# learningmatter-mit/surface-sampling

Measured on AMD Instinct MI355X. Metric: MC energy-evaluations/sec (SrTiO3(001) ~250-atom slabs, 3-model PaiNN ensemble E+F incl. neighbor list), higher is better.
Workload: dtype f32 via fp16x2-split MFMA (3 products), fp32 accumulate; neighbor decisions f64; 1 GPU; SrTiO3(001) PaiNN x3, 256 batched independent chains per GPU (BASELINE configs[3]), 248-272 atoms/chain; chains_per_gpu=256, atoms_per_gpu=66503, edges_per_gpu=2747786, slots_per_gpu=2836316, models=3, streams_per_gpu=2, parallelism=one GPU, no collective

## Files before the change

### surface-sampling_amd/csrc/api_batch.hip

```cpp
#include <cmath>

#include "vssr_internal.h"

namespace vssr {

static void cell_host_setup(const double *cell, const uint8_t *pbc, double cutoff, double inv[9], int nimg[3],
                            bool &ok) {
    const double *a = cell, *b = cell + 3, *c = cell + 6;
    double bc[3] = {b[1] * c[2] - b[2] * c[1], b[2] * c[0] - b[0] * c[2], b[0] * c[1] - b[1] * c[0]};
    double ca[3] = {c[1] * a[2] - c[2] * a[1], c[2] * a[0] - c[0] * a[2], c[0] * a[1] - c[1] * a[0]};
    double ab[3] = {a[1] * b[2] - a[2] * b[1], a[2] * b[0] - a[0] * b[2], a[0] * b[1] - a[1] * b[0]};
    double vol = a[0] * bc[0] + a[1] * bc[1] + a[2] * bc[2];
    ok = true;
    for (int x = 0; x < 9; ++x) inv[x] = 0.0;
    nimg[0] = nimg[1] = nimg[2] = 0;
    if (!(pbc[0] || pbc[1] || pbc[2])) return;
    if (std::fabs(vol) < 1e-12) { ok = false; return; }
    for (int x = 0; x < 3; ++x) { inv[x] = bc[x] / vol; inv[3 + x] = ca[x] / vol; inv[6 + x] = ab[x] / vol; }
    double hgt[3] = {std::fabs(vol) / std::sqrt(bc[0] * bc[0] + bc[1] * bc[1] + bc[2] * bc[2]),
                     std::fabs(vol) / std::sqrt(ca[0] * ca[0] + ca[1] * ca[1] + ca[2] * ca[2]),
                     std::fabs(vol) / std::sqrt(ab[0] * ab[0] + ab[1] * ab[1] + ab[2] * ab[2])};
    for (int k = 0; k < 3; ++k)
        if (pbc[k]) nimg[k] = (int)std::floor(cutoff / hgt[k]) + 1;
}
// ... 247 lines not shown
        return set_err(h, VSSR_E_BADARG, "bad FIRE parameters");
    VSSR_HIP(h, hipSetDevice(h->device));
    h->relax_regrows = 0;
    h->last_want = want | VSSR_WANT_FORCES;
    if (int rc = relax_fire(h, *params, fixed, want)) return rc;
    return relax_finish(h, pos_out, n_steps, converged);
}

static int relax_finish(vssr_handle *h, double *pos_out, int32_t *n_steps, uint8_t *converged) {
    VSSR_HIP(h, hipStreamSynchronize(h->stream));
    h->prof.collect();
    if (pos_out) VSSR_HIP(h, hipMemcpy(pos_out, h->d_pos.p, sizeof(double) * 3 * h->n_atoms, hipMemcpyDeviceToHost));
    if (n_steps) VSSR_HIP(h, hipMemcpy(n_steps, h->d_relax_steps.p, sizeof(int) * h->n_cfg, hipMemcpyDeviceToHost));
    if (converged) VSSR_HIP(h, hipMemcpy(converged, h->d_relax_conv.p, (size_t)h->n_cfg, hipMemcpyDeviceToHost));
    return VSSR_OK;
}

int vssr_profile_enable(vssr_handle *h, int enable) {
    if (int rc = check_kind(h, KINDS_EVAL, __func__)) return rc;
    VSSR_HIP(h, hipStreamSynchronize(h->stream));
    h->prof.collect();
    h->prof.enabled = enable != 0;
    return VSSR_OK;
}
int vssr_profile_reset(vssr_handle *h) {
    if (int rc = check_kind(h, KINDS_EVAL, __func__)) return rc;
    VSSR_HIP(h, hipStreamSynchronize(h->stream));
    h->prof.reset();
    return VSSR_OK;
}
int vssr_profile_read(vssr_handle *h, int32_t cap, const char **names, int64_t *launches, double *total_ms,
                      int32_t *n_out) {
    if (!h || !n_out) return VSSR_E_BADARG;
    if (int rc = check_kind(h, KINDS_EVAL, __func__)) return rc;
    VSSR_HIP(h, hipStreamSynchronize(h->stream));
    h->prof.collect();
    int n = 0;
    for (int k = 0; k < KC_COUNT && n < cap; ++k) {
        if (names) names[n] = kKernelClassNames[k];
        if (launches) launches[n] = h->prof.launches[k];
        if (total_ms) total_ms[n] = h->prof.total_ms[k];
        ++n;
    }
    *n_out = n;
    return VSSR_OK;
}

int vssr_batch_stats(vssr_handle *h, int64_t *n_atoms, int64_t *n_edges, int64_t *n_slots) {
    if (int rc = check_kind(h, KINDS_EVAL, __func__)) return rc;
    if (!h->ran) return set_err(h, VSSR_E_STATE, "no completed run");
    if (h->graph_partial)
        return set_err(h, VSSR_E_STATE, "the resident graph covers only the chains of the last relaxation iteration: run the batch once (vssr_batch_run) first");
    int rc = sync_and_check(h);
    if (rc) return rc;
    if (n_atoms) *n_atoms = h->n_atoms;
    if (n_edges) *n_edges = h->h_counters[1];
    if (n_slots) *n_slots = h->h_counters[0];
    return VSSR_OK;
}

int vssr_batch_neighbors(vssr_handle *h, int64_t cap, int32_t *ei, int32_t *ej, int32_t *eS, float *er,
                         int64_t *n_edges) {
    if (!h || !n_edges) return VSSR_E_BADARG;
    if (int rc = check_kind(h, KINDS_EVAL, __func__)) return rc;
    if (!h->ran) return set_err(h, VSSR_E_STATE, "no completed run");
    if (h->graph_partial)
        return set_err(h, VSSR_E_STATE, "the resident graph covers only the chains of the last relaxation iteration: run the batch once (vssr_batch_run) first");
    int rc = sync_and_check(h);
    if (rc) return rc;
    const int N = h->n_atoms;
    const int64_t slots = h->h_counters[0];
    *n_edges = h->h_counters[1];
    if (!ei && !ej && !eS && !er) return VSSR_OK;
    std::vector<int> row(N + 1), S(slots), wrap((size_t)3 * N);
    std::vector<float4> edge(slots);
    VSSR_HIP(h, hipMemcpy(row.data(), h->d_row_start.p, sizeof(int) * (N + 1), hipMemcpyDeviceToHost));
    VSSR_HIP(h, hipMemcpy(S.data(), h->d_edge_S.p, sizeof(int) * slots, hipMemcpyDeviceToHost));
    VSSR_HIP(h, hipMemcpy(edge.data(), h->d_edge.p, sizeof(float4) * slots, hipMemcpyDeviceToHost));
    VSSR_HIP(h, hipMemcpy(wrap.data(), h->d_wrap.p, sizeof(int) * 3 * N, hipMemcpyDeviceToHost));
    int64_t n = 0;
    for (int i = 0; i < N; ++i)
        for (int e = row[i]; e < row[i + 1]; ++e) {
            int j;
            memcpy(&j, &edge[e].w, sizeof(int));
            if (j < 0) continue;
            if (n < cap) {
                if (ei) ei[n] = i;
                if (ej) ej[n] = j;
                if (eS)
                    for (int k = 0; k < 3; ++k)
                        eS[3 * n + k] = (((S[e] >> (8 * k)) & 255) - 128) + wrap[3 * i + k] - wrap[3 * j + k];
                if (er) { er[3 * n] = edge[e].x; er[3 * n + 1] = edge[e].y; er[3 * n + 2] = edge[e].z; }
            }
            ++n;
        }
    return VSSR_OK;
}

int vssr_batch_device_results(vssr_handle *h, const float **energy, const float **energy_std) {
    if (int rc = check_kind(h, KINDS_EVAL, __func__)) return rc;
    if (!h->ran || h->kind != Kind::PAINN) return set_err(h, VSSR_E_STATE, "no completed PaiNN run");
    if (energy) *energy = h->d_energy.as<float>();
    if (energy_std) *energy_std = h->d_energy_std.as<float>();
    return VSSR_OK;
}

int vssr_batch_device_results_f64(vssr_handle *h, const double **energy, const double **energy_std) {
    if (int rc = check_kind(h, KINDS_EVAL, __func__)) return rc;
    if (!h->ran || h->kind != Kind::PAINN) return set_err(h, VSSR_E_STATE, "no completed PaiNN run");
    if (energy) *energy = h->d_energy64.as<double>();
    if (energy_std) *energy_std = h->d_energy64.as<double>() + h->n_cfg;
    return VSSR_OK;
}

int vssr_batch_energy_f64(vssr_handle *h, double *energy, double *energy_std, double *energy_models) {
    if (int rc = check_kind(h, KINDS_EVAL, __func__)) return rc;
    if (!h->ran) return set_err(h, VSSR_E_STATE, "vssr_batch_energy_f64 before a run");
    VSSR_HIP(h, hipSetDevice(h->device));
    int rc = sync_and_check(h);
    if (rc) return rc;
    const size_t B = h->n_cfg, M = h->n_models;
    if (is_analytic(h)) {
        if (energy) VSSR_HIP(h, hipMemcpy(energy, h->d_pot_e.p, sizeof(double) * B, hipMemcpyDeviceToHost));
        if (energy_models) VSSR_HIP(h, hipMemcpy(energy_models, h->d_pot_e.p, sizeof(double) * B, hipMemcpyDeviceToHost));
        if (energy_std) for (size_t b = 0; b < B; ++b) energy_std[b] = 0.0;
        return VSSR_OK;
    }
    const double *src = h->d_energy64.as<double>();
    if (energy) VSSR_HIP(h, hipMemcpy(energy, src, sizeof(double) * B, hipMemcpyDeviceToHost));
    if (energy_std) VSSR_HIP(h, hipMemcpy(energy_std, src + B, sizeof(double) * B, hipMemcpyDeviceToHost));
    if (energy_models) VSSR_HIP(h, hipMemcpy(energy_models, src + 2 * B, sizeof(double) * B * M, hipMemcpyDeviceToHost));
    return VSSR_OK;
}

int vssr_batch_results_f64(vssr_handle *h, double *energy, double *energy_atoms, double *forces) {
    if (int rc = check_kind(h, KINDS_EVAL, __func__)) return rc;
    if (!is_analytic(h)) return set_err(h, VSSR_E_STATE, "vssr_batch_results_f64 needs an fp64 potential (Tersoff / EAM / SW / pair handle)");
    if (!h->ran) return set_err(h, VSSR_E_STATE, "vssr_batch_results_f64 before a run");
    VSSR_HIP(h, hipSetDevice(h->device));
    if (forces && !(h->last_want & VSSR_WANT_FORCES))
        return set_err(h, VSSR_E_STATE, "forces requested, but the last run was asked for energies only");
    int rc = sync_and_check(h);
    if (rc) return rc;
    const size_t B = h->n_cfg, N = h->n_atoms;
    if (energy) VSSR_HIP(h, hipMemcpy(energy, h->d_pot_e.p, sizeof(double) * B, hipMemcpyDeviceToHost));
    if (energy_atoms) VSSR_HIP(h, hipMemcpy(energy_atoms, h->d_pot_ea.p, sizeof(double) * N, hipMemcpyDeviceToHost));
    if (forces) VSSR_HIP(h, hipMemcpy(forces, h->d_pot_f.p, sizeof(double) * 3 * N, hipMemcpyDeviceToHost));
    return VSSR_OK;
}

int vssr_device_context(vssr_handle *h, int32_t *device, void **stream, const int32_t **overflow_flag) {
    if (int rc = check_kind(h, KINDS_EVAL, __func__)) return rc;
    if (device) *device = h->device;
    if (stream) *stream = (void *)h->stream;
    if (overflow_flag) *overflow_flag = h->d_counters.p ? h->d_counters.as<int>() + 2 : nullptr;
    return VSSR_OK;
}

int vssr_batch_traj_configure(vssr_handle *h, int32_t record_interval) {
    if (int rc = check_kind(h, KINDS_EVAL, __func__)) return rc;
    if (record_interval < 0) return set_err(h, VSSR_E_BADARG, "record_interval must be >= 0");
    h->traj_interval = record_interval;
    return VSSR_OK;
}

int vssr_batch_traj_read(vssr_handle *h, int32_t cap_records, int32_t *n_records, double *pos, float *forces, double *energy,
                         int32_t *max_records) {
    if (int rc = check_kind(h, KINDS_EVAL, __func__)) return rc;
    if (max_records) *max_records = h->traj_records;
    if (!h->traj_records) {
        if (n_records || pos || forces || energy) return set_err(h, VSSR_E_STATE, "the last relaxation recorded no trajectory");
        return VSSR_OK;
    }
    if (!n_records && !pos && !forces && !energy) return VSSR_OK;
    if (h->traj_B != h->n_cfg || h->traj_N != h->n_atoms) return set_err(h, VSSR_E_STATE, "the recorded trajectory belongs to another batch");
    if (cap_records < h->traj_records) return set_err(h, VSSR_E_BADARG, "trajectory buffers hold %d records, %d are needed", cap_records, h->traj_records);
    VSSR_HIP(h, hipSetDevice(h->device));
    VSSR_HIP(h, hipStreamSynchronize(h->stream));
    const size_t R = h->traj_records, N3 = (size_t)3 * h->traj_N, B = h->traj_B;
    if (n_records) VSSR_HIP(h, hipMemcpy(n_records, h->d_traj_n.p, sizeof(int) * B, hipMemcpyDeviceToHost));
    if (pos) VSSR_HIP(h, hipMemcpy(pos, h->d_traj_pos.p, sizeof(double) * N3 * R, hipMemcpyDeviceToHost));
    if (forces) VSSR_HIP(h, hipMemcpy(forces, h->d_traj_f.p, sizeof(float) * N3 * R, hipMemcpyDeviceToHost));
    if (energy) VSSR_HIP(h, hipMemcpy(energy, h->d_traj_e.p, sizeof(double) * B * R, hipMemcpyDeviceToHost));
    return VSSR_OK;
}

int vssr_batch_embedding(vssr_handle *h, int32_t model, float *dst, int64_t cap, int64_t *n_out) {
    if (int rc = check_kind(h, KINDS_EVAL, __func__)) return rc;
    if (!h->ran || h->kind != Kind::PAINN) return set_err(h, VSSR_E_STATE, "no completed PaiNN run");
    if (model < -1 || model >= h->n_models) return set_err(h, VSSR_E_BADARG, "model index out of range");
    if (h->graph_partial)
        return set_err(h, VSSR_E_STATE, "the resident activations cover only the chains of the last relaxation iteration: run the batch once (vssr_batch_run) first");
    VSSR_HIP(h, hipSetDevice(h->device));
    int rc = sync_and_check(h);
    if (rc) return rc;
    const size_t per_model = (size_t)h->n_atoms * h->feat_dim, n = model < 0 ? per_model * h->n_models : per_model;
    if (n_out) *n_out = (int64_t)n;
    if (!dst) return VSSR_OK;
    if ((int64_t)n > cap) return set_err(h, VSSR_E_BADARG, "embedding buffer too small (%lld < %zu floats)", (long long)cap, n);
    const float *src = h->sv.s_in[h->num_conv] + (model < 0 ? 0 : (size_t)model * per_model);
    VSSR_HIP(h, hipMemcpy(dst, src, n * sizeof(float), hipMemcpyDeviceToHost));
    return VSSR_OK;
}

int vssr_batch_stress(vssr_handle *h, double *stress, double *stress_std) {
    if (int rc = check_kind(h, KINDS_EVAL, __func__)) return rc;
    if (!h->ran || !evaluator(h).stress) return set_err(h, VSSR_E_STATE, "no completed PaiNN, Tersoff, EAM or Stillinger-Weber run");
    if (!(h->last_want & VSSR_WANT_FORCES))
        return set_err(h, VSSR_E_STATE, "stress needs the edge gradients of a run that produced forces; the last run was asked for energies only");
    if (h->graph_partial)
        return set_err(h, VSSR_E_STATE, "the resident graph covers only the chains of the last relaxation iteration: run the batch once (vssr_batch_run) first");
    VSSR_HIP(h, hipSetDevice(h->device));
    int rc = sync_and_check(h);
    if (rc) return rc;
    rc = evaluator(h).stress(h);
    if (rc) return rc;
    VSSR_HIP(h, hipStreamSynchronize(h->stream));
    const size_t n = 6 * (size_t)h->n_cfg;
    if (stress) VSSR_HIP(h, hipMemcpy(stress, h->d_stress.p, sizeof(double) * n, hipMemcpyDeviceToHost));
    if (stress_std) VSSR_HIP(h, hipMemcpy(stress_std, h->d_stress.as<double>() + n, sizeof(double) * n, hipMemcpyDeviceToHost));
    return VSSR_OK;
}

int vssr_batch_saturated(vssr_handle *h, uint8_t *flags, int32_t *n_flagged) {
    if (int rc = check_kind(h, KINDS_EVAL, __func__)) return rc;
    if (!h->ran) return set_err(h, VSSR_E_STATE, "no completed run");
    VSSR_HIP(h, hipSetDevice(h->device));
    int count = 0;
    if (h->kind == Kind::PAINN) {
        if (!h->h_sat_valid || (int)h->h_sat.size() != h->n_cfg) {
            int rc = sync_and_check(h);
            if (rc) return rc;
            h->h_sat.resize(h->n_cfg);
            VSSR_HIP(h, hipMemcpy(h->h_sat.data(), h->d_sat_out.p, sizeof(unsigned) * h->n_cfg, hipMemcpyDeviceToHost));
            h->h_sat_valid = true;
        }
        const std::vector<unsigned> &f = h->h_sat;
        for (int b = 0; b < h->n_cfg; ++b) {
            if (flags) flags[b] = f[b] ? 1 : 0;
            count += f[b] ? 1 : 0;
        }
    } else if (flags) {
        memset(flags, 0, (size_t)h->n_cfg);
    }
    if (n_flagged) *n_flagged = count;
    return VSSR_OK;
}

int vssr_debug_capacity(vssr_handle *h, int32_t slots_per_atom, int32_t tight, int32_t *n_regrows) {
    if (int rc = check_kind(h, KINDS_EVAL, __func__)) return rc;
    if (slots_per_atom > 0) {
        h->cap_per_atom = slots_per_atom;
        h->cm_cap_per_atom = 0;
        h->slot_cap = 0;
    }
    if (tight >= 0) h->cap_tight = tight != 0;
    if (n_regrows) *n_regrows = h->relax_regrows;
    return VSSR_OK;
}

int vssr_batch_relax_counts(vssr_handle *h, int64_t *lockstep_evaluations, int64_t *chain_evaluations) {
    if (int rc = check_kind(h, KINDS_EVAL, __func__)) return rc;
    if (lockstep_evaluations) *lockstep_evaluations = h->relax_lockstep;
    if (chain_evaluations) *chain_evaluations = h->relax_chain_evals;
    return VSSR_OK;
}

int vssr_debug_read(vssr_handle *h, const char *name, int32_t model, float *dst, int64_t cap, int64_t *n_out) {
    if (!h || !name || !n_out) return VSSR_E_BADARG;
    if (int rc = check_kind(h, KINDS_EVAL, __func__)) return rc;
    if (!h->ran || h->kind != Kind::PAINN) return set_err(h, VSSR_E_STATE, "no completed PaiNN run");
    if (model < 0 || model >= h->n_models) return set_err(h, VSSR_E_BADARG, "model index out of range");
    if (h->painn_general) return set_err(h, VSSR_E_STATE, "per-layer intermediates are not kept by the general-width PaiNN path");
    if (h->graph_partial)
        return set_err(h, VSSR_E_STATE, "the resident graph covers only the chains of the last relaxation iteration: run the batch once (vssr_batch_run) first");
    int rc = sync_and_check(h);
    if (rc) return rc;
    const size_t N = h->n_atoms;
    const StateView &sv = h->sv;
    const float *src = nullptr;
    size_t per_atom = 0;
    std::string nm(name);
    auto layer_of = [&](const char *prefix) -> int {
        size_t pl = strlen(prefix);
        if (nm.compare(0, pl, prefix) != 0 || nm.size() != pl + 1) return -1;
        int l = nm[pl] - '0';
        return (l >= 0 && l < h->num_conv) ? l : -1;
    };
    int l;
    if ((l = layer_of("phi")) >= 0) {
        if (l == 0 && h->l0_used)
            return set_err(h, VSSR_E_STATE, "phi0 is not materialised (layer-0 species factorisation is active)");
        src = sv.phi[l]; per_atom = F3;
    }
    else if ((l = layer_of("s_msg")) >= 0) { src = sv.s_msg[l]; per_atom = F; }
    else if ((l = layer_of("v_msg")) >= 0) { src = sv.v_msg[l]; per_atom = F3; }
    else if ((l = layer_of("s_upd")) >= 0) { src = sv.s_in[l + 1]; per_atom = F; }
    else if ((l = layer_of("v_upd")) >= 0) {
        if (l == h->num_conv - 1 && !h->debug_keep)
            return set_err(h, VSSR_E_STATE, "v_upd of the last block is not materialised (nothing consumes it; create the handle with VSSR_DEBUG_KEEP=1)");
        src = sv.v_in[l + 1]; per_atom = F3;
    }
    else if (nm == "e_atom") { src = sv.e_atom; per_atom = 1; }
    else if (nm == "sbar_msg0") { src = sv.sbar_msg_l0; per_atom = F; }
    else if (nm == "vbar_msg0") { src = sv.vbar_msg; per_atom = F3; }
    else return set_err(h, VSSR_E_BADARG, "unknown intermediate '%s'", name);
    size_t n = N * per_atom;
    *n_out = (int64_t)n;
    if (!dst) return VSSR_OK;
    if ((int64_t)n > cap) return set_err(h, VSSR_E_BADARG, "buffer too small for '%s'", name);
    VSSR_HIP(h, hipMemcpy(dst, src + (size_t)model * n, n * sizeof(float), hipMemcpyDeviceToHost));
    return VSSR_OK;
}

}
```

### surface-sampling_amd/csrc/api_painn.hip

```cpp
#include <cmath>

#include "vssr_internal.h"

namespace vssr {

static void transpose(const float *src, int rows, int cols, float *dst) {
    for (int r = 0; r < rows; ++r)
        for (int c = 0; c < cols; ++c) dst[(size_t)c * rows + r] = src[(size_t)r * cols + c];
}

static int upload_weights(vssr_handle *h, const vssr_painn_config *cfg) {
    const int M = cfg->n_models, L = cfg->num_conv, R = cfg->n_rbf, H = cfg->readout_hidden, NE = cfg->n_embed;
    const size_t per_layer = (size_t)F * F + F + (size_t)F3 * F + F3 + (size_t)F3 * R + F3 + 2 * (size_t)F * F +
                             (size_t)F * 2 * F + F + (size_t)F3 * F + F3;
    const size_t blob_len = (size_t)NE * F + L * per_layer + (size_t)H * F + H + H + 1;
    if (cfg->weights_len != blob_len)
        return set_err(h, VSSR_E_BADARG, "weights_len %llu does not match the layout (%zu floats)",
                       (unsigned long long)cfg->weights_len, blob_len);
    const size_t t_per_layer = (size_t)F * F + (size_t)F * F3 + 2 * (size_t)F * F + (size_t)2 * F * F + (size_t)F * F3;
    const size_t img_len = blob_len + L * t_per_layer + (size_t)F * H;
    std::vector<float> img(img_len * M);
    std::vector<ModelW> table(M);
    if (h->weights.ensure(img.size() * sizeof(float)))
        return set_err(h, VSSR_E_NOMEM, "weights: out of device memory");
    float *dbase = h->weights.as<float>();
    const size_t node16_per_layer = (size_t)22 * F * F;
    const size_t node16_readout = (size_t)2 * H * F;
    std::vector<unsigned> node16(node16_per_layer * L * M + node16_readout * M);
    for (int m = 0; m < M; ++m) {
        float *hb = img.data() + (size_t)m * img_len;
        float *db = dbase + (size_t)m * img_len;
        memcpy(hb, cfg->weights[m], blob_len * sizeof(float));
        for (size_t t = 0; t < blob_len; ++t)
            if (!std::isfinite(hb[t])) return set_err(h, VSSR_E_BADARG, "model %d: non-finite weight", m);
        ModelW &W = table[m];
        size_t o = 0, to = blob_len;
        auto take = [&](size_t n) { size_t r = o; o += n; return r; };
        auto taket = [&](size_t n) { size_t r = to; to += n; return r; };
        W.embed = db + take((size_t)NE * F);
        for (int l = 0; l < L; ++l) {
            LayerW &Lw = W.layer[l];
            size_t w1 = take((size_t)F * F), b1 = take(F), w2 = take((size_t)F3 * F), b2 = take(F3);
            size_t wd = take((size_t)F3 * R), bd = take(F3), u = take((size_t)F * F), v = take((size_t)F * F);
            size_t w3 = take((size_t)F * 2 * F), b3 = take(F), w4 = take((size_t)F3 * F), b4 = take(F3);
            size_t w1t = taket((size_t)F * F), w2t = taket((size_t)F * F3), ut = taket((size_t)F * F);
            size_t vt = taket((size_t)F * F), w3t = taket((size_t)2 * F * F), w4t = taket((size_t)F * F3);
            transpose(hb + w1, F, F, hb + w1t);
            transpose(hb + w2, F3, F, hb + w2t);
            transpose(hb + u, F, F, hb + ut);
            transpose(hb + v, F, F, hb + vt);
            transpose(hb + w3, F, 2 * F, hb + w3t);
            transpose(hb + w4, F3, F, hb + w4t);
            Lw.W1 = db + w1; Lw.W1t = db + w1t; Lw.b1 = db + b1;
            Lw.W2 = db + w2; Lw.W2t = db + w2t; Lw.b2 = db + b2;
            Lw.Wd = db + wd; Lw.bd = db + bd;
            Lw.U = db + u; Lw.Ut = db + ut; Lw.V = db + v; Lw.Vt = db + vt;
            Lw.W3 = db + w3; Lw.W3t = db + w3t; Lw.b3 = db + b3;
            Lw.W4 = db + w4; Lw.W4t = db + w4t; Lw.b4 = db + b4;
            {
                std::vector<float> uvt((size_t)F * 2 * F);
                for (int g = 0; g < F; ++g)
                    for (int k = 0; k < F; ++k) {
                        uvt[(size_t)g * 2 * F + k] = hb[u + (size_t)k * F + g];
                        uvt[(size_t)g * 2 * F + F + k] = hb[v + (size_t)k * F + g];
                    }
                unsigned *q = node16.data() + ((size_t)m * L + l) * node16_per_layer;
                auto put16 = [&](const float *src, int rows, int K) {
                    pack_mfma_tiles16(src, rows, K, q);
                    q += (size_t)rows * K;
                };
                put16(hb + w1, F, F); put16(hb + w2, F3, F); put16(hb + u, F, F); put16(hb + v, F, F);
                put16(hb + w3, F, 2 * F); put16(hb + w4, F3, F); put16(hb + w1t, F, F); put16(hb + w2t, F, F3);
                put16(hb + w4t, F, F3); put16(hb + w3t, 2 * F, F); put16(uvt.data(), F, 2 * F);
            }
        }
        size_t w5 = take((size_t)H * F), b5 = take(H), w6 = take(H), b6 = take(1);
        size_t w5t = taket((size_t)F * H);
        transpose(hb + w5, H, F, hb + w5t);
        W.W5 = db + w5; W.W5t = db + w5t; W.b5 = db + b5; W.w6 = db + w6; W.b6 = db + b6;
        if (H % 32 == 0) {
            unsigned *q = node16.data() + node16_per_layer * L * M + node16_readout * m;
            pack_mfma_tiles16(hb + w5, H, F, q);
            pack_mfma_tiles16(hb + w5t, F, H, q + (size_t)H * F);
        }
    }
    VSSR_HIP(h, hipMemcpy(dbase, img.data(), img.size() * sizeof(float), hipMemcpyHostToDevice));
    {
        if (h->node16.ensure(node16.size() * sizeof(unsigned))) return set_err(h, VSSR_E_NOMEM, "split node weights");
        VSSR_HIP(h, hipMemcpy(h->node16.p, node16.data(), node16.size() * sizeof(unsigned), hipMemcpyHostToDevice));
        for (int m = 0; m < M; ++m)
            for (int l = 0; l < L; ++l) {
                LayerW &Lw = table[m].layer[l];
                const uint4 *q = h->node16.as<uint4>() + ((size_t)m * L + l) * node16_per_layer / 4;
                auto next = [&](int rows, int K) { const uint4 *r = q; q += (size_t)rows * K / 4; return r; };
                Lw.qW1 = next(F, F); Lw.qW2 = next(F3, F); Lw.qU = next(F, F); Lw.qV = next(F, F);
                Lw.qW3 = next(F, 2 * F); Lw.qW4 = next(F3, F); Lw.qW1t = next(F, F); Lw.qW2t = next(F, F3);
                Lw.qW4t = next(F, F3); Lw.qW3t = next(2 * F, F); Lw.qUVt = next(F, 2 * F);
            }
        for (int m = 0; m < M; ++m) {
            const uint4 *q = h->node16.as<uint4>() + (node16_per_layer * L * M + node16_readout * m) / 4;
            table[m].qW5 = q;
            table[m].qW5t = q + (size_t)H * F / 4;
        }
    }
    {
        const size_t per_layer16 = (size_t)F3 * 4 * 8;
        std::vector<unsigned> w16(per_layer16 * L * M);
        for (int m = 0; m < M; ++m) {
            const float *hb = img.data() + (size_t)m * img_len;
            size_t o = (size_t)NE * F;
            for (int l = 0; l < L; ++l) {
                const float *Wd = hb + o + (size_t)F * F + F + (size_t)F3 * F + F3;
                build_wd16(Wd, Wd + (size_t)F3 * 20, w16.data() + ((size_t)m * L + l) * per_layer16);
                o += per_layer;
            }
        }
        if (h->wd16.ensure(w16.size() * sizeof(unsigned))) return set_err(h, VSSR_E_NOMEM, "split filter weights");
        VSSR_HIP(h, hipMemcpy(h->wd16.p, w16.data(), w16.size() * sizeof(unsigned), hipMemcpyHostToDevice));
        for (int m = 0; m < M; ++m)
            for (int l = 0; l < L; ++l)
                table[m].layer[l].wd16 = h->wd16.as<uint4>() + ((size_t)m * L + l) * per_layer16 / 4;
    }
    {
        const size_t per_model = (size_t)NE * 2 * 24 * F;
        std::vector<float> A(per_model * M), At(per_model * M);
        for (int m = 0; m < M; ++m) {
            const float *hb = img.data() + (size_t)m * img_len;
            size_t o = (size_t)NE * F;
            const float *W1 = hb + o; o += (size_t)F * F;
            const float *b1 = hb + o; o += F;
            const float *W2 = hb + o; o += (size_t)F3 * F;
            const float *b2 = hb + o; o += F3;
            const float *Wd = hb + o; o += (size_t)F3 * R;
            const float *bd = hb + o;
            l0_build_tables(hb, W1, b1, W2, b2, Wd, bd, NE, A.data() + per_model * m, At.data() + per_model * m);
        }
        const size_t pk = l0_packed_dwords(NE);
        std::vector<unsigned> A16(pk * M), At16(pk * M);
        for (int m = 0; m < M; ++m) l0_pack_tables(A.data() + per_model * m, NE, A16.data() + pk * m, At16.data() + pk * m);
        if (h->d_l0A.ensure(A16.size() * sizeof(unsigned)) || h->d_l0At.ensure(At16.size() * sizeof(unsigned)))
            return set_err(h, VSSR_E_NOMEM, "layer-0 tables");
        VSSR_HIP(h, hipMemcpy(h->d_l0A.p, A16.data(), A16.size() * sizeof(unsigned), hipMemcpyHostToDevice));
        VSSR_HIP(h, hipMemcpy(h->d_l0At.p, At16.data(), At16.size() * sizeof(unsigned), hipMemcpyHostToDevice));
    }
    if (h->model_table.ensure(sizeof(ModelW) * M)) return set_err(h, VSSR_E_NOMEM, "model table");
    VSSR_HIP(h, hipMemcpy(h->model_table.p, table.data(), sizeof(ModelW) * M, hipMemcpyHostToDevice));
    return VSSR_OK;
}

}

using namespace vssr;

extern "C" {

int vssr_create(const vssr_painn_config *cfg, vssr_handle **out) {
    if (!cfg || !out) return set_err(nullptr, VSSR_E_BADARG, "null argument");
    *out = nullptr;
    if (cfg->struct_size != sizeof(vssr_painn_config))
        return set_err(nullptr, VSSR_E_BADARG, "vssr_painn_config size mismatch (%u vs %zu)", cfg->struct_size,
                       sizeof(vssr_painn_config));
    if (cfg->feat_dim < 16 || cfg->feat_dim > 256 || cfg->feat_dim % 16 != 0 || cfg->n_rbf < 1 || cfg->n_rbf > 32)
        return set_err(nullptr, VSSR_E_BADARG,
                       "feat_dim must be a multiple of 16 in 16..256 and n_rbf in 1..32 (got %d, %d)", cfg->feat_dim, cfg->n_rbf);
    if (cfg->n_models < 1 || cfg->n_models > MAX_MODELS || cfg->num_conv < 1 || cfg->num_conv > MAX_LAYERS ||
        cfg->readout_hidden < 1 || cfg->readout_hidden > F || cfg->n_embed < 1 || !cfg->weights ||
        !(cfg->cutoff > 0) || !(cfg->model_units_per_ev > 0))
        return set_err(nullptr, VSSR_E_BADARG, "bad PaiNN configuration");
    if (cfg->excl_vol && (cfg->excl_power < 1 || cfg->excl_power > 64 || !(cfg->excl_sigma > 0)))
        return set_err(nullptr, VSSR_E_BADARG, "excluded volume: power %d (1 .. 64) / sigma %g out of range", cfg->excl_power,
                       (double)cfg->excl_sigma);
    return create_handle(Kind::PAINN, cfg->device, out, [cfg](vssr_handle *h) {
        h->n_models = cfg->n_models; h->n_rbf = cfg->n_rbf; h->num_conv = cfg->num_conv; h->n_embed = cfg->n_embed;
        h->readout_hidden = cfg->readout_hidden; h->cutoff = cfg->cutoff; h->excl_vol = cfg->excl_vol;
        h->excl_power = cfg->excl_power; h->excl_sigma = cfg->excl_sigma; h->units_per_ev = cfg->model_units_per_ev;
        h->feat_dim = cfg->feat_dim;
        h->painn_general = !(cfg->feat_dim == F && cfg->n_rbf == 20);
        if (const char *e = getenv("VSSR_PAINN_PATH")) h->painn_general = h->painn_general || strcmp(e, "general") == 0;
        int rc = VSSR_OK;
        if (h->painn_general) {
            h->l0_enabled = 0;
            rc = painn_gen_upload(h, cfg);
        } else {
            rc = upload_weights(h, cfg);
            if (!rc) rc = node_mfma_init(h);
            if (!rc) rc = edge_mfma_init(h);
            if (!rc) rc = l0_mfma_init(h);
        }
        if (const char *e = getenv("VSSR_EDGE_IMPL")) h->edge_impl = (strcmp(e, "gather") == 0) ? 0 : 1;
        if (const char *e = getenv("VSSR_L0_FACTORISE")) h->l0_enabled = h->painn_general ? 0 : atoi(e);
        if (const char *e = getenv("VSSR_UPD_SAVE")) h->upd_save = atoi(e);
        if (const char *e = getenv("VSSR_DEBUG_KEEP")) h->debug_keep = atoi(e);
        if (const char *e = getenv("VSSR_EDGE_FS16_MAX")) h->fs16_max_atoms = atoi(e);
        if (const char *e = getenv("VSSR_EDGE_FS8_MAX")) h->fs8_max_atoms = atoi(e);
        if (const char *e = getenv("VSSR_EDGE_BWD_MPASS")) h->bwd_multi_pass = atoi(e);
        if (const char *e = getenv("VSSR_EDGE_SUB_CHUNK")) { const int c = atoi(e); if (c >= 8) { h->sub_chunk_fwd = c; h->sub_chunk_bwd = c; } }
        if (const char *e = getenv("VSSR_EDGE_FWD_2PASS")) { const int w = atoi(e); h->fwd_two_pass = (w == 8 || w == 16) ? w : w ? 16 : 0; }
        if (!rc && cfg->offset_per_z) {
            h->has_offset = true;
            h->offset_const = cfg->offset_const;
            if (h->offset_per_z.ensure(sizeof(double) * cfg->n_embed)) rc = set_err(h, VSSR_E_NOMEM, "offset table");
            else if (hipMemcpy(h->offset_per_z.p, cfg->offset_per_z, sizeof(double) * cfg->n_embed,
                               hipMemcpyHostToDevice) != hipSuccess)
                rc = set_err(h, VSSR_E_DEVICE, "offset table upload failed");
        }
        return rc;
    });
}

}
```

### surface-sampling_amd/csrc/mfma16.h

```cpp
#ifndef VSSR_MFMA16_H
#define VSSR_MFMA16_H
#include "vssr_internal.h"

namespace vssr {

typedef float f32x4 __attribute__((ext_vector_type(4)));
typedef float f32x2 __attribute__((ext_vector_type(2)));
typedef unsigned u32x4 __attribute__((ext_vector_type(4)));
typedef unsigned u32x2 __attribute__((ext_vector_type(2)));
typedef _Float16 f16x8 __attribute__((ext_vector_type(8)));
typedef _Float16 f16x2 __attribute__((ext_vector_type(2)));

constexpr int TA = 32;
constexpr int NW = 8;
constexpr int NTHREADS = 64 * NW;
constexpr int PADH = 8;

#ifndef VSSR_FAST_SIGMOID
#define VSSR_FAST_SIGMOID 1
#endif
__device__ __forceinline__ float sigm(float x) {
#if VSSR_FAST_SIGMOID && defined(__HIP_DEVICE_COMPILE__)
    constexpr float C_HI = -1.44269502162933349609375f;
    constexpr float C_LO = -1.9259629911266175e-08f;
    constexpr float LN2 = 0.693147182464599609375f;
    x = fmaxf(x, -87.f);
    const float y = x * C_HI;
    const float r = fmaf(x, C_LO, fmaf(x, C_HI, -y));
    const float e = __builtin_amdgcn_exp2f(y);
    const float en = fmaf(e, r * LN2, e);
    return __builtin_amdgcn_rcpf(1.f + en);
#else
    return 1.f / (1.f + expf(-x));
#endif
}
__device__ __forceinline__ float swish(float x) { return x * sigm(x); }
__device__ __forceinline__ float dswish(float x) {
    float sg = sigm(x);
    return sg * fmaf(x, 1.f - sg, 1.f);
}

__device__ __forceinline__ u32x4 gload4u(const uint4 *p) {
#if defined(__HIP_DEVICE_COMPILE__)
    typedef const u32x4 __attribute__((address_space(1))) *gptr;
    return *reinterpret_cast<gptr>(reinterpret_cast<uintptr_t>(p));
#else
    return *reinterpret_cast<const u32x4 *>(p);
#endif
}

struct Planes {
    _Float16 *h, *l;
    int ld;
};
__device__ __forceinline__ Planes make_planes(_Float16 *base, int rows, int K) {
    return Planes{base, base + (size_t)rows * (K + PADH), K + PADH};
}
constexpr int plane_halves(int rows, int K) { return 2 * rows * (K + PADH); }

#ifndef VSSR_SAT_TRACK
#define VSSR_SAT_TRACK 1
#endif
enum { SAT_ACC = 0, SAT_COOP = 1, SAT_ANY = 2 };
struct SatTrack {
    float acc_lo = 0.f, acc_hi = 0.f, coop_lo = 0.f, coop_hi = 0.f;
    unsigned rows = 0u;
    static constexpr float LIM = 65504.f;
    template <int LAYOUT>
    __device__ __forceinline__ void see(int row, float a, float b, float c, float d) {
        if (!VSSR_SAT_TRACK) return;
        if (LAYOUT == SAT_ANY) {
            const float mx = fmaxf(fmaxf(fabsf(a), fabsf(b)), fmaxf(fabsf(c), fabsf(d)));
            rows |= mx > LIM ? 1u << (row & (TA - 1)) : 0u;
            return;
        }
        auto upd = [&](float m) { return fmaxf(fmaxf(fmaxf(fmaxf(m, fabsf(a)), fabsf(b)), fabsf(c)), fabsf(d)); };
        const bool upper = (row >> 4) & 1;
        if (LAYOUT == SAT_ACC) { acc_lo = upper ? acc_lo : upd(acc_lo); acc_hi = upper ? upd(acc_hi) : acc_hi; }
        else { coop_lo = upper ? coop_lo : upd(coop_lo); coop_hi = upper ? upd(coop_hi) : coop_hi; }
    }
    __device__ __forceinline__ void commit(const ActiveView &av, int a0, int N) const {
        if (!VSSR_SAT_TRACK || !av.sat) return;
        const float worst = fmaxf(fmaxf(acc_lo, acc_hi), fmaxf(coop_lo, coop_hi));
        if (!(worst > LIM) && rows == 0u) return;
        auto raise = [&](int row) {
            const int c = av.atom_cfg[min(a0 + (row & (TA - 1)), N - 1)];
            if (av.chain(c)) atomicOr(av.sat + c, 1u);
        };
        int tid = threadIdx.x;
        asm volatile("" : "+v"(tid));
        const int r = tid & 15, rho = (tid & (NTHREADS - 1)) >> 5;
        if (acc_lo > LIM) raise(r);
        if (acc_hi > LIM) raise(16 + r);
        if (coop_lo > LIM) raise(rho);
        if (coop_hi > LIM) raise(16 + rho);
        for (unsigned m = rows; m; m &= m - 1u) raise(__builtin_ctz(m));
    }
};

struct SatNone {
    template <int LAYOUT>
    __device__ __forceinline__ void see(int, float, float, float, float) {}
};

template <int LAYOUT = SAT_ACC, class Sat>
__device__ __forceinline__ void store_split4(const Planes &P, int row, int col, float4 v, Sat &sat) {
    sat.template see<LAYOUT>(row, v.x, v.y, v.z, v.w);
    const f32x2 a = {__builtin_amdgcn_fmed3f(v.x, -65504.f, 65504.f), __builtin_amdgcn_fmed3f(v.y, -65504.f, 65504.f)};
    const f32x2 b = {__builtin_amdgcn_fmed3f(v.z, -65504.f, 65504.f), __builtin_amdgcn_fmed3f(v.w, -65504.f, 65504.f)};
    const f16x2 ha = __builtin_convertvector(a, f16x2), hb = __builtin_convertvector(b, f16x2);
    const f16x2 la = __builtin_convertvector(a - __builtin_convertvector(ha, f32x2), f16x2);
    const f16x2 lb = __builtin_convertvector(b - __builtin_convertvector(hb, f32x2), f16x2);
    *reinterpret_cast<u32x2 *>(P.h + row * P.ld + col) = (u32x2){__builtin_bit_cast(unsigned, ha), __builtin_bit_cast(unsigned, hb)};
    *reinterpret_cast<u32x2 *>(P.l + row * P.ld + col) = (u32x2){__builtin_bit_cast(unsigned, la), __builtin_bit_cast(unsigned, lb)};
}

template <int LAYOUT = SAT_ACC, class Sat>
__device__ __forceinline__ void store_split4(const Planes &P, int row, int col, f32x4 v, Sat &sat) {
    store_split4<LAYOUT>(P, row, col, make_float4(v[0], v[1], v[2], v[3]), sat);
}

template <int NROWS, class RowPtr, class Sat>
__device__ __forceinline__ void load_rows_split(const Planes &P, int col0, RowPtr rowptr, Sat &sat) {
    constexpr int NIT = NROWS * (F / 4) / NTHREADS;
    static_assert(NROWS * (F / 4) % NTHREADS == 0, "tile load must divide evenly");
    float4 v[NIT];
#pragma unroll
    for (int it = 0; it < NIT; ++it) {
        const int idx = threadIdx.x + it * NTHREADS;
        v[it] = *reinterpret_cast<const float4 *>(rowptr(idx >> 5) + 4 * (idx & 31));
    }
#pragma unroll
    for (int it = 0; it < NIT; ++it) {
        const int idx = threadIdx.x + it * NTHREADS;
        store_split4<SAT_COOP>(P, idx >> 5, col0 + 4 * (idx & 31), v[it], sat);
    }
}
template <int NROWS, class RowPtr>
__device__ __forceinline__ void rows_request(RowPtr rowptr, float4 (&v)[NROWS * (F / 4) / NTHREADS]) {
    constexpr int NIT = NROWS * (F / 4) / NTHREADS;
#pragma unroll
    for (int it = 0; it < NIT; ++it) {
        const int idx = threadIdx.x + it * NTHREADS;
        v[it] = *reinterpret_cast<const float4 *>(rowptr(idx >> 5) + 4 * (idx & 31));
    }
}
template <int NROWS, class Sat>
__device__ __forceinline__ void rows_store_split(const Planes &P, int col0, const float4 (&v)[NROWS * (F / 4) / NTHREADS],
                                                 Sat &sat) {
    constexpr int NIT = NROWS * (F / 4) / NTHREADS;
#pragma unroll
    for (int it = 0; it < NIT; ++it) {
        const int idx = threadIdx.x + it * NTHREADS;
        store_split4<SAT_COOP>(P, idx >> 5, col0 + 4 * (idx & 31), v[it], sat);
    }
}

constexpr int FT = F + 4;
template <int NROWS, class Fn>
__device__ __forceinline__ void stage_rows(const float *T, Fn fn) {
    constexpr int NIT = NROWS * (F / 4) / NTHREADS;
    static_assert(NROWS * (F / 4) % NTHREADS == 0, "tile pass must divide evenly");
#pragma unroll
    for (int it = 0; it < NIT; ++it) {
        const int idx = threadIdx.x + it * NTHREADS, row = idx >> 5, c4 = idx & 31;
        fn(row, 4 * c4, *reinterpret_cast<const float4 *>(T + row * FT + 4 * c4));
    }
}

template <int NROWS, class Ld, class St>
__device__ __forceinline__ void stage_rows_residual(const float *T, Ld ld, St st) {
    constexpr int NIT = NROWS * (F / 4) / NTHREADS;
    static_assert(NROWS * (F / 4) % NTHREADS == 0, "tile pass must divide evenly");
    float4 r[NIT];
#pragma unroll
    for (int it = 0; it < NIT; ++it) {
        const int idx = threadIdx.x + it * NTHREADS;
        r[it] = ld(idx >> 5, 4 * (idx & 31));
    }
#pragma unroll
    for (int it = 0; it < NIT; ++it) {
        const int idx = threadIdx.x + it * NTHREADS, row = idx >> 5, c4 = idx & 31;
        st(row, 4 * c4, *reinterpret_cast<const float4 *>(T + row * FT + 4 * c4), r[it]);
    }
}

__device__ __forceinline__ f32x4 mfma16(u32x4 a, u32x4 b, f32x4 c) {
    return __builtin_amdgcn_mfma_f32_16x16x32_f16(__builtin_bit_cast(f16x8, a), __builtin_bit_cast(f16x8, b), c, 0, 0, 0);
}

struct LaneGeo {
    int w, col0, r;
    __device__ __forceinline__ LaneGeo() {
        const int lane = threadIdx.x & 63;
        w = threadIdx.x >> 6;
        col0 = 16 * w + 4 * (lane >> 4);
        r = lane & 15;
    }
    __device__ __forceinline__ int row(int t) const { return 16 * t + r; }
};
__device__ __forceinline__ f32x4 gload4f(const float *p) {
#if defined(__HIP_DEVICE_COMPILE__)
    typedef const f32x4 __attribute__((address_space(1))) *gptr;
    return *reinterpret_cast<gptr>(reinterpret_cast<uintptr_t>(p));
#else
    return *reinterpret_cast<const f32x4 *>(p);
#endif
}

__device__ __forceinline__ float gload1f(const float *p) {
#if defined(__HIP_DEVICE_COMPILE__)
    typedef const float __attribute__((address_space(1))) *gptr;
    return *reinterpret_cast<gptr>(reinterpret_cast<uintptr_t>(p));
#else
    return *p;
#endif
}

}
#endif
```

### surface-sampling_amd/csrc/painn.hip

```cpp
#include "vssr_internal.h"

namespace vssr {

constexpr int T = NODE_TILE;
constexpr int RB = 21;
constexpr int ECHUNK = 16;
constexpr float PI_F = 3.14159265358979323846f;

__device__ inline float sigmoidf_(float x) { return 1.f / (1.f + expf(-x)); }
__device__ inline float swishf_(float x) { return x * sigmoidf_(x); }
__device__ inline float dswishf_(float x) {
    float sg = sigmoidf_(x);
    return sg * fmaf(x, 1.f - sg, 1.f);
}

__global__ void __launch_bounds__(128) k_embed(int N, const int *__restrict__ Z, const ModelW *__restrict__ MW,
                                               float *__restrict__ s0, float *__restrict__ v0) {
    int i = blockIdx.x, m = blockIdx.y, f = threadIdx.x;
    const ModelW &W = MW[m];
    size_t a = (size_t)m * N + i;
    s0[a * F + f] = W.embed[(size_t)Z[i] * F + f];
    v0[(a * 3 + 0) * F + f] = 0.f;
    v0[(a * 3 + 1) * F + f] = 0.f;
    v0[(a * 3 + 2) * F + f] = 0.f;
// ... 240 lines not shown
                dpart = fmaf(pc_a * q, dA, dpart);
            }
            float mc = pc_c * wC;
            red[e][0][f] = dpart;
            red[e][1][f] = mc * vb0;
            red[e][2][f] = mc * vb1;
            red[e][3][f] = mc * vb2;
        }
        __syncthreads();
        if (f < ne * 4) {
            int e = f >> 2, comp = f & 3;
            float tot = 0.f;
            for (int k = 0; k < F; ++k) tot += red[e][comp][k];
            tots[e][comp] = tot;
        }
        __syncthreads();
        if (f < ne && S.j[f] >= 0) {
            float d = S.u[f][3];
            float u0 = -S.u[f][0], u1 = -S.u[f][1], u2 = -S.u[f][2];
            float db = tots[f][0];
            if (L0 && excl_vol) db -= (float)excl_power * powf(excl_sigma / d, (float)excl_power) / d;
            float b0 = tots[f][1], b1 = tots[f][2], b2 = tots[f][3];
            float dot = fmaf(b2, u2, fmaf(b1, u1, b0 * u0));
            float g0 = fmaf(db, u0, (b0 - dot * u0) / d);
            float g1 = fmaf(db, u1, (b1 - dot * u1) / d);
            float g2 = fmaf(db, u2, (b2 - dot * u2) / d);
            if (accumulate) {
                float4 old = gb[e0 + f];
                g0 += old.x; g1 += old.y; g2 += old.z;
            }
            gb[e0 + f] = make_float4(g0, g1, g2, 0.f);
        }
        __syncthreads();
    }
    if (!L0) {
        phibar[ac * F3 + f] = fmaf(vc2, az, fmaf(vc1, ay, vc0 * ax));
        phibar[ac * F3 + F + f] = accb;
        phibar[ac * F3 + 2 * F + f] = accc;
        vbar_in[(ac * 3 + 0) * F + f] = fmaf(pc_a, ax, vbar_msg[(ac * 3 + 0) * F + f]);
        vbar_in[(ac * 3 + 1) * F + f] = fmaf(pc_a, ay, vbar_msg[(ac * 3 + 1) * F + f]);
        vbar_in[(ac * 3 + 2) * F + f] = fmaf(pc_a, az, vbar_msg[(ac * 3 + 2) * F + f]);
    }
}

__global__ void __launch_bounds__(256)
k_reduce_gpart(int M, int n_groups, int layer_sets, GraphView G, const int *__restrict__ counters, const float *__restrict__ P,
               float4 *__restrict__ gbar, long long slot_cap, int uniform_slices) {
    if (counters[2]) return;
    const int per_set = n_groups / layer_sets;
    long long s0, s1;
    int slices;
    if (uniform_slices) {
        s0 = 0; s1 = counters[0]; slices = uniform_slices;
    } else {
        const int b = blockIdx.x;
        if (!G.act.chain(b)) return;
        slices = edge_bclass_slices(G.chain_class[b]);
        if (slices == 1) return;
        s0 = G.row_start[G.cfg_start[b]]; s1 = G.row_start[G.cfg_start[b + 1]];
    }
    const long long first = uniform_slices ? (long long)blockIdx.x * blockDim.x : (long long)blockIdx.y * blockDim.x;
    const long long step = uniform_slices ? (long long)gridDim.x * blockDim.x : (long long)gridDim.y * blockDim.x;
    for (long long slot = s0 + first + threadIdx.x; slot < s1; slot += step)
        for (int m = 0; m < M; ++m) {
            float4 acc = gbar[(size_t)m * slot_cap + slot];
            for (int k = 0; k < layer_sets; ++k)
                for (int grp = 0; grp < slices; ++grp) {
                    const float *p = P + ((size_t)(m * n_groups + k * per_set + grp) * slot_cap + slot) * 3;
                    acc.x += p[0]; acc.y += p[1]; acc.z += p[2];
                }
            gbar[(size_t)m * slot_cap + slot] = acc;
        }
}

__global__ void k_reduce_gbar_groups_uniform(int M, int n_groups, const int *__restrict__ counters, float4 *__restrict__ gbar,
                                             long long gbar_stride) {
    const long long slot = (long long)blockIdx.x * blockDim.x + threadIdx.x;
    if (counters[2] || slot >= counters[0]) return;
    for (int m = 0; m < M; ++m) {
        float4 *g0 = gbar + (size_t)(m * n_groups) * gbar_stride + slot;
        float4 acc = *g0;
        for (int grp = 1; grp < n_groups; ++grp) {
            const float4 v = g0[(size_t)grp * gbar_stride];
            acc.x += v.x; acc.y += v.y; acc.z += v.z;
        }
        *g0 = acc;
    }
}

__global__ void __launch_bounds__(256)
k_reduce_gbar_groups(int M, int n_groups, int layer_sets, GraphView G, const int *__restrict__ counters, float4 *__restrict__ gbar,
                     long long gbar_stride) {
    if (counters[2]) return;
    const int b = blockIdx.x;
    if (!G.act.chain(b)) return;
    const int slices = edge_bclass_slices(G.chain_class[b]);
    if (slices == 1) return;
    const int per_set = n_groups / layer_sets;
    const int s0 = G.row_start[G.cfg_start[b]], s1 = G.row_start[G.cfg_start[b + 1]];
    for (int slot = s0 + blockIdx.y * blockDim.x + threadIdx.x; slot < s1; slot += gridDim.y * blockDim.x)
        for (int m = 0; m < M; ++m) {
            float4 *g0 = gbar + (size_t)(m * n_groups) * gbar_stride + slot;
            float4 acc = *g0;
            for (int k = 0; k < layer_sets; ++k)
                for (int grp = k ? 0 : 1; grp < slices; ++grp) {
                    const float4 v = g0[(size_t)(k * per_set + grp) * gbar_stride];
                    acc.x += v.x; acc.y += v.y; acc.z += v.z;
                }
            *g0 = acc;
        }
}

__global__ void __launch_bounds__(256)
k_finalize_forces(int N, int M, GraphView G, const int *__restrict__ counters,
                  const float4 *__restrict__ gbar, long long gbar_model_stride, double units_per_ev,
                  float *__restrict__ forces, float *__restrict__ forces_std) {
    const int lane = threadIdx.x & 63;
    const int c = blockIdx.x * (blockDim.x >> 6) + (threadIdx.x >> 6);
    if (c >= N || counters[2] || !G.act.atom(c)) return;
    const int e0 = G.row_start[c], e1 = G.row_start[c + 1];
    double fm[3] = {0, 0, 0}, f2[3] = {0, 0, 0};
    for (int m = 0; m < M; ++m) {
        float g0 = 0.f, g1 = 0.f, g2 = 0.f;
        const float4 *gb = gbar + (size_t)m * gbar_model_stride;
        for (int e = e0 + lane; e < e1; e += 64) {
            const int r = G.rev[e];
            if (r < 0) continue;
            const float4 a = gb[e], b = gb[r];
            g0 += a.x - b.x; g1 += a.y - b.y; g2 += a.z - b.z;
        }
        g0 = wave_sum_f32(g0); g1 = wave_sum_f32(g1); g2 = wave_sum_f32(g2);
        double f[3] = {-(double)g0 / units_per_ev, -(double)g1 / units_per_ev, -(double)g2 / units_per_ev};
        for (int x = 0; x < 3; ++x) { fm[x] += f[x]; f2[x] += f[x] * f[x]; }
    }
    if (lane < 3) {
        const int x = lane;
        const double fmx = x == 0 ? fm[0] : x == 1 ? fm[1] : fm[2], f2x = x == 0 ? f2[0] : x == 1 ? f2[1] : f2[2];
        double mu = fmx / M;
        double var = f2x / M - mu * mu;
        forces[3 * c + x] = (float)mu;
        if (forces_std) forces_std[3 * c + x] = (float)sqrt(var > 0 ? var : 0.0);
    }
}

__global__ void __launch_bounds__(256)
k_stress(int M, GraphView G, const int *__restrict__ counters, const float4 *__restrict__ gbar, long long gbar_model_stride,
         const double *__restrict__ cell, double units_per_ev, double *__restrict__ stress, double *__restrict__ stress_std) {
    __shared__ double red[9][256];
    const int b = blockIdx.x, tid = threadIdx.x;
    if (counters[2]) return;
    const int s0 = G.row_start[G.cfg_start[b]], s1 = G.row_start[G.cfg_start[b + 1]];
    const double *c = cell + 9 * (size_t)b;
    const double vol = fabs(c[0] * (c[4] * c[8] - c[5] * c[7]) - c[1] * (c[3] * c[8] - c[5] * c[6]) + c[2] * (c[3] * c[7] - c[4] * c[6]));
    double mean[6] = {0, 0, 0, 0, 0, 0}, sq[6] = {0, 0, 0, 0, 0, 0};
    for (int m = 0; m < M; ++m) {
        const float4 *gb = gbar + (size_t)m * gbar_model_stride;
        double w[9] = {0, 0, 0, 0, 0, 0, 0, 0, 0};
        for (int e = s0 + tid; e < s1; e += 256) {
            const float4 r = G.edge[e];
            if (__float_as_int(r.w) < 0) continue;
            const float4 g = gb[e];
            const double gx = g.x, gy = g.y, gz = g.z, rx = r.x, ry = r.y, rz = r.z;
            w[0] -= gx * rx; w[1] -= gx * ry; w[2] -= gx * rz;
            w[3] -= gy * rx; w[4] -= gy * ry; w[5] -= gy * rz;
            w[6] -= gz * rx; w[7] -= gz * ry; w[8] -= gz * rz;
        }
        for (int k = 0; k < 9; ++k) red[k][tid] = w[k];
        __syncthreads();
        for (int s = 128; s > 0; s >>= 1) {
            if (tid < s)
                for (int k = 0; k < 9; ++k) red[k][tid] += red[k][tid + s];
            __syncthreads();
        }
        if (tid == 0) {
            const double f = 1.0 / (units_per_ev * vol);
            const double v[6] = {red[0][0] * f, red[4][0] * f, red[8][0] * f, 0.5 * (red[5][0] + red[7][0]) * f,
                                 0.5 * (red[2][0] + red[6][0]) * f, 0.5 * (red[1][0] + red[3][0]) * f};
            for (int k = 0; k < 6; ++k) { mean[k] += v[k]; sq[k] += v[k] * v[k]; }
        }
        __syncthreads();
    }
    if (tid == 0)
        for (int k = 0; k < 6; ++k) {
            const double mu = mean[k] / M, var = sq[k] / M - mu * mu;
            stress[6 * (size_t)b + k] = mu;
            if (stress_std) stress_std[6 * (size_t)b + k] = sqrt(var > 0 ? var : 0.0);
        }
}

__global__ void __launch_bounds__(256)
k_finalize_energy(int N, int M, const unsigned char *__restrict__ active, const int *__restrict__ cfg_start, const int *__restrict__ Z,
                  const float *__restrict__ e_atom, double units_per_ev, const double *__restrict__ offset_per_z,
                  double offset_const, float *__restrict__ energy, float *__restrict__ energy_std,
                  float *__restrict__ energy_models, double *__restrict__ energy64, float *__restrict__ e_atoms_mean,
                  unsigned *__restrict__ sat, unsigned *__restrict__ sat_out) {
    __shared__ double red[256];
    __shared__ double em[MAX_MODELS];
    const int b = blockIdx.x, tid = threadIdx.x;
    if (active && !active[b]) return;
    const int a0 = cfg_start[b], a1 = cfg_start[b + 1];
    double off = 0.0;
    if (offset_per_z) {
        for (int i = a0 + tid; i < a1; i += blockDim.x) off += offset_per_z[Z[i]];
    }
    red[tid] = off;
    __syncthreads();
    for (int s = 128; s > 0; s >>= 1) {
        if (tid < s) red[tid] += red[tid + s];
        __syncthreads();
    }
    double offset = offset_per_z ? red[0] + offset_const : 0.0;
    __syncthreads();
    for (int m = 0; m < M; ++m) {
        double acc = 0.0;
        for (int i = a0 + tid; i < a1; i += blockDim.x) acc += (double)e_atom[(size_t)m * N + i];
        red[tid] = acc;
        __syncthreads();
        for (int s = 128; s > 0; s >>= 1) {
            if (tid < s) red[tid] += red[tid + s];
            __syncthreads();
        }
        if (tid == 0) em[m] = red[0] / units_per_ev + offset;
        __syncthreads();
    }
    if (tid == 0) {
        double mu = 0, var = 0;
        for (int m = 0; m < M; ++m) mu += em[m];
        mu /= M;
        for (int m = 0; m < M; ++m) var += (em[m] - mu) * (em[m] - mu);
        energy[b] = (float)mu;
        energy_std[b] = (float)sqrt(var / M);
        const int B = gridDim.x;
        energy64[b] = mu;
        energy64[B + b] = sqrt(var / M);
        for (int m = 0; m < M; ++m) energy64[(size_t)2 * B + (size_t)b * M + m] = em[m];
        sat_out[b] = (sat[b] != 0u || !isfinite((float)mu)) ? 1u : 0u;
        sat[b] = 0u;
        for (int m = 0; m < M; ++m) energy_models[(size_t)b * M + m] = (float)em[m];
    }
    for (int i = a0 + tid; i < a1; i += blockDim.x) {
        double acc = 0;
        for (int m = 0; m < M; ++m) acc += (double)e_atom[(size_t)m * N + i];
        e_atoms_mean[i] = (float)(acc / M / units_per_ev);
    }
}

static int gbar_layer_sets(const vssr_handle *h) { return h->gbar_mode == 2 ? h->num_conv - 1 : h->gbar_mode == 1 && h->num_conv > 2 ? h->num_conv - 1 : 1; }
int painn_gbar_groups(const vssr_handle *h) {
    if (h->num_conv < 2) return 1;
    const int per_set = h->n_bclass[EDGE_BCLASS_FS4] ? edge_class_groups(EDGE_BCLASS_FS4)
                        : h->n_bclass[EDGE_BCLASS_FS8] ? edge_class_groups(EDGE_BCLASS_FS8)
                        : (h->n_bclass[EDGE_BCLASS_FS16] || h->n_bclass[EDGE_BCLASS_FS16P]) ? edge_class_groups(EDGE_BCLASS_FS16) : 1;
    return per_set > 1 ? per_set * gbar_layer_sets(h) : 1;
}

int painn_alloc_state(vssr_handle *h) {
    const size_t N = h->n_atoms, M = h->n_models, L = h->num_conv;
    const size_t nS = M * N * F, nV = 3 * nS, nP = 3 * nS;
    size_t floats = (L + 1) * (nS + nV) + L * nP + L * (nS + nV) + M * N
                    + 2 * (nS + nV) + nP;
    if (h->d_state.ensure(floats * sizeof(float)))
        return set_err(h, VSSR_E_NOMEM, "activation arena (%zu MB): out of device memory", floats * 4 >> 20);
    float *p = h->d_state.as<float>();
    StateView &sv = h->sv;
    sv.n_atoms = (int)N;
    sv.n_models = (int)M;
    for (size_t l = 0; l <= L; ++l) { sv.s_in[l] = p; p += nS; sv.v_in[l] = p; p += nV; }
    for (size_t l = 0; l < L; ++l) {
        sv.phi[l] = p; p += nP;
        sv.s_msg[l] = p; p += nS;
        sv.v_msg[l] = p; p += nV;
    }
    sv.e_atom = p; p += M * N;
    sv.sbar = p; p += nS;
    sv.vbar = p; p += nV;
    sv.sbar_msg = p; p += nS;
    sv.vbar_msg = p; p += nV;
    sv.phibar = p; p += nP;
    if (h->upd_save && readout_mfma_supported(h->readout_hidden) &&
        h->d_upd_save.ensure(update_save_bytes((int)N, (int)M) * L))
        return set_err(h, VSSR_E_NOMEM, "forward intermediates of the update blocks: out of device memory");
    const size_t groups = (size_t)painn_gbar_groups(h);
    const bool compact = h->gbar_mode == 2 && groups > 1;
    if (h->d_gbar.ensure(sizeof(float4) * M * (compact ? 1 : groups) * (size_t)h->slot_cap) ||
        (compact && h->d_gpart.ensure(sizeof(float) * 3 * M * groups * (size_t)h->slot_cap + 256)))
        return set_err(h, VSSR_E_NOMEM, "edge-gradient buffer: out of device memory");
    sv.gbar = h->d_gbar.as<float4>();
    return painn_alloc_results(h);
}

int painn_alloc_results(vssr_handle *h) {
    const size_t N = h->n_atoms, M = h->n_models;
    if (h->d_energy.ensure(sizeof(float) * h->n_cfg) || h->d_energy_std.ensure(sizeof(float) * h->n_cfg) ||
        h->d_energy_models.ensure(sizeof(float) * h->n_cfg * M) || h->d_energy64.ensure(sizeof(double) * h->n_cfg * (2 + M)) ||
        h->d_forces.ensure(sizeof(float) * 3 * N) ||
        h->d_forces_std.ensure(sizeof(float) * 3 * N) || h->d_e_atoms.ensure(sizeof(float) * N))
        return set_err(h, VSSR_E_NOMEM, "result buffers: out of device memory");
    if (h->d_sat.bytes < sizeof(unsigned) * h->n_cfg || h->d_sat_out.bytes < sizeof(unsigned) * h->n_cfg) {
        if (h->d_sat.ensure(sizeof(unsigned) * h->n_cfg) || h->d_sat_out.ensure(sizeof(unsigned) * h->n_cfg))
            return set_err(h, VSSR_E_NOMEM, "saturation flags: out of device memory");
        VSSR_HIP(h, hipMemsetAsync(h->d_sat.p, 0, h->d_sat.bytes, h->stream));
        VSSR_HIP(h, hipMemsetAsync(h->d_sat_out.p, 0, h->d_sat_out.bytes, h->stream));
    }
    return VSSR_OK;
}

int painn_run(vssr_handle *h, uint32_t want) {
    if (h->painn_general) return painn_gen_run(h, want);
    const int N = h->n_atoms, M = h->n_models, L = h->num_conv, H = h->readout_hidden;
    hipStream_t st = h->stream;
    h->h_sat_valid = false;
    int rc = build_neighbors(h, (double)h->cutoff);
    if (rc) return rc;
    rc = painn_alloc_state(h);
    if (rc) return rc;
    StateView &sv = h->sv;
    sv.e_excl = h->d_excl.as<float>();
    GraphView G;
    G.n_atoms = N;
    G.n_cfg = h->n_cfg;
    G.atom_cfg = h->d_atom_cfg.as<int>();
    G.cfg_start = h->d_cfg_start.as<int>();
    G.row_start = h->d_row_start.as<int>();
    G.deg = h->d_deg.as<int>();
    G.edge = h->d_edge.as<float4>();
    G.rev = h->d_rev.as<int>();
    G.erec = h->d_erec.as<float4>();
    G.rho = h->d_rho.as<float>();
    G.dist2 = h->d_dist.as<float2>();
    G.rho16 = h->d_rho16.as<uint4>();
    G.drho16 = h->d_drho16.as<uint4>();
    G.zslot = h->d_zslot.as<unsigned char>();
    G.bundle = h->d_bundle.as<int4>();
    G.chain_class = h->d_chain_class.as<unsigned char>();
    G.act = ActiveView{h->active_mask, h->d_atom_cfg.as<int>(), h->d_sat.as<unsigned>()};
    const ActiveView &av = G.act;
    const ModelW *MW = h->model_table.as<ModelW>();
    const int *counters = h->d_counters.as<int>();
    const int *Z = h->d_Z.as<int>();
    dim3 blk(128);
    dim3 g_atom(N, M), g_tile((N + T - 1) / T, M);
    Profiler &P = h->prof;
    const bool l0_fact = h->l0_enabled && h->l0_nz > 0;
    const int n_groups = painn_gbar_groups(h);
    const int layer_sets = n_groups > 1 ? gbar_layer_sets(h) : 1;
    const bool compact = h->gbar_mode == 2 && n_groups > 1;
    const int fin_groups = compact ? 1 : n_groups;
    const int *cls_list[EDGE_MFMA_CLASSES];
    const int *bcls_list[EDGE_MFMA_BCLASSES];
    {
        int o = 0;
        for (int c = 0; c < EDGE_MFMA_CLASSES; o += h->n_class[c], ++c) cls_list[c] = h->d_class_list.as<int>() + o;
        for (int c = 0; c < EDGE_MFMA_BCLASSES; o += h->n_bclass[c], ++c) bcls_list[c] = h->d_class_list.as<int>() + o;
    }
    const int n_gather = h->n_class[EDGE_CLASS_GATHER];
    const bool keep = h->upd_save && (want & VSSR_WANT_FORCES) && readout_mfma_supported(H);
    auto save_of = [&](int l) -> void * { return keep ? (char *)h->d_upd_save.p + update_save_bytes(N, M) * (size_t)l : nullptr; };
    h->l0_used = l0_fact;

    if (!l0_fact) {
        P.begin(KC_EMBED, st);
        hipLaunchKernelGGL(k_embed, g_atom, blk, 0, st, N, Z, MW, sv.s_in[0], sv.v_in[0]);
        P.end(st);
    }
    for (int l = 0; l < L; ++l) {
        if (l == 0 && l0_fact) {
            P.begin(KC_L0_FWD, st);
            rc = l0_run_forward(h, G, sv.s_msg[0], sv.v_msg[0]);
            if (rc) return rc;
            P.end(st);
            P.begin(KC_UPDATE_FWD, st);
            launch_update_fwd_mfma(st, N, M, l, av, MW, sv.s_msg[l], sv.v_msg[l], sv.s_in[l + 1],
                                   (l + 1 < L || h->debug_keep) ? sv.v_in[l + 1] : nullptr, l + 1 < L ? sv.phi[l + 1] : nullptr, save_of(l));
            P.end(st);
            continue;
        }
        if (l == 0) {
            P.begin(KC_MSG_MLP, st);
            launch_msg_mlp_mfma(st, N, M, l, av, MW, sv.s_in[l], sv.phi[l]);
            P.end(st);
        }
        P.begin(KC_EDGE_FWD, st);
        if (l == 0)
            hipLaunchKernelGGL(k_edge_fwd<true>, g_atom, blk, 0, st, N, l, MW, G, counters, h->cutoff, h->excl_vol,
                               h->excl_sigma, h->excl_power, sv.s_in[l], sv.v_in[l], sv.phi[l], sv.s_msg[l],
                               sv.v_msg[l], -1);
        else {
            for (int cls = 0; cls < EDGE_MFMA_CLASSES; ++cls)
                launch_edge_fwd_mfma(st, cls, N, cls_list[cls], h->n_class[cls], M, l, h->max_class_atoms[cls], MW, G, counters,
                                     (int)(h->slot_cap - 1), sv.s_in[l], sv.v_in[l], sv.phi[l], sv.s_msg[l], sv.v_msg[l],
                                     (cls == EDGE_CLASS_FS4 && h->fwd_two_pass) ? h->d_bundle_sub.as<int4>() : (const int4 *)nullptr,
                                     h->fwd_two_pass, h->sub_chunk_fwd ? h->sub_chunk_fwd : sub_chunk_max(h->fwd_two_pass));
            if (n_gather)
                hipLaunchKernelGGL(k_edge_fwd<false>, g_atom, blk, 0, st, N, l, MW, G, counters, h->cutoff, h->excl_vol,
                                   h->excl_sigma, h->excl_power, sv.s_in[l], sv.v_in[l], sv.phi[l], sv.s_msg[l],
                                   sv.v_msg[l], (int)EDGE_BCLASS_GATHER);
        }
        P.end(st);
        P.begin(KC_UPDATE_FWD, st);
        launch_update_fwd_mfma(st, N, M, l, av, MW, sv.s_msg[l], sv.v_msg[l], sv.s_in[l + 1],
                               (l + 1 < L || h->debug_keep) ? sv.v_in[l + 1] : nullptr, l + 1 < L ? sv.phi[l + 1] : nullptr, save_of(l));
        P.end(st);
    }
    const bool fused = readout_mfma_supported(H);
    const bool want_forces = (want & VSSR_WANT_FORCES) != 0;
    const float *e_excl = h->excl_vol ? sv.e_excl : (const float *)nullptr;
    if (!(fused && want_forces)) {
        P.begin(KC_READOUT, st);
        if (fused) launch_readout_mfma(st, N, M, av, MW, sv.s_in[L], e_excl, sv.e_atom);
        else
            hipLaunchKernelGGL(k_readout, g_tile, blk, 0, st, N, H, av, MW, sv.s_in[L], sv.e_excl, h->excl_vol, sv.e_atom,
                               sv.sbar);
        P.end(st);
    }

    if (want_forces) {
        float *sb_buf[2] = {sv.sbar_msg, sv.sbar};
        for (int l = L - 1; l >= 0; --l) {
            float *sbar_msg_l = fused ? sb_buf[(L - 1 - l) & 1] : sv.sbar_msg;
            const float *sbar_msg_up = sb_buf[(L - l) & 1];
            P.begin(KC_UPDATE_BWD, st);
            if (!fused)
                launch_update_bwd_mfma(st, N, M, l, 0, (int)(l == L - 1), av, MW, sv.s_msg[l], sv.v_msg[l], sv.sbar, sv.vbar,
                                       nullptr, nullptr, nullptr, nullptr, sbar_msg_l, sv.vbar_msg, nullptr);
            else if (l == L - 1)
                launch_update_bwd_mfma(st, N, M, l, 1, 1, av, MW, sv.s_msg[l], sv.v_msg[l], nullptr, sv.vbar, sv.s_in[L], nullptr,
                                       e_excl, sv.e_atom, sbar_msg_l, sv.vbar_msg, save_of(l));
            else
                launch_update_bwd_mfma(st, N, M, l, 2, 0, av, MW, sv.s_msg[l], sv.v_msg[l], sbar_msg_up, sv.vbar, sv.s_in[l + 1],
                                       sv.phibar, nullptr, nullptr, sbar_msg_l, sv.vbar_msg, save_of(l));
            P.end(st);
            sv.sbar_msg_l0 = sbar_msg_l;
            P.begin((l == 0 && l0_fact) ? KC_L0_BWD : KC_EDGE_BWD, st);
            int accumulate = (l != L - 1);
            if (l == 0 && l0_fact) {
                rc = l0_run_reverse(h, G, (int)(L == 1), (int)compact, sbar_msg_l, sv.vbar_msg, sv.gbar, (long long)h->slot_cap,
                                    fin_groups);
                if (rc) return rc;
            } else if (l == 0)
                hipLaunchKernelGGL(k_edge_bwd<true>, g_atom, blk, 0, st, N, l, accumulate, MW, G, counters,
                                   h->cutoff, h->excl_vol, h->excl_sigma, h->excl_power, sv.v_in[l], sv.phi[l],
                                   sbar_msg_l, sv.vbar_msg, sv.phibar, sv.vbar, sv.gbar,
                                   (long long)h->slot_cap * fin_groups, -1, (int)compact);
            else {
                if ((l == L - 1 || layer_sets > 1) && !compact && h->n_cfg > n_gather)
                    return set_err(h, VSSR_E_STATE, "matrix-pipe reverse kernels need the compact partial-gradient records");
                for (int cls = 0; cls < EDGE_MFMA_BCLASSES; ++cls)
                    launch_edge_bwd_mfma(st, cls, N, bcls_list[cls], h->n_bclass[cls], M, l, (int)(l == L - 1 || layer_sets > 1),
                                         h->max_bclass_atoms[cls], MW, G, counters, (int)(h->slot_cap - 1), sv.v_in[l], sv.phi[l],
                                         sbar_msg_l, sv.vbar_msg, sv.phibar, sv.vbar,
                                         compact ? h->d_gpart.as<float>() : reinterpret_cast<float *>(sv.gbar), (long long)h->slot_cap,
                                         n_groups, layer_sets > 1 ? (L - 1 - l) * (n_groups / layer_sets) : 0, compact ? 3 : 4,
                                         cls == EDGE_BCLASS_FS16P ? h->d_bundle_subb.as<int4>() : (const int4 *)nullptr,
                                         h->sub_chunk_bwd ? h->sub_chunk_bwd : sub_chunk_max_bwd());
                if (n_gather)
                    hipLaunchKernelGGL(k_edge_bwd<false>, g_atom, blk, 0, st, N, l, accumulate, MW, G, counters,
                                       h->cutoff, h->excl_vol, h->excl_sigma, h->excl_power, sv.v_in[l], sv.phi[l],
                                       sbar_msg_l, sv.vbar_msg, sv.phibar, sv.vbar, sv.gbar,
                                       (long long)h->slot_cap * fin_groups, (int)EDGE_BCLASS_GATHER, 0);
            }
            P.end(st);
            if (l > 0 && !fused) {
                P.begin(KC_MSG_MLP_BWD, st);
                launch_msg_mlp_bwd_mfma(st, N, M, l, av, MW, sv.s_in[l], sv.phibar, sv.sbar_msg, sv.sbar);
                P.end(st);
            }
        }
    }
    P.begin(KC_FINALIZE, st);
    if (want & VSSR_WANT_FORCES) {
#ifdef ABL_LDS_FORCE
        if (compact) {
        } else if (false) {
#else
        if (compact) {
#endif
            const int uni = h->active_mask ? 0 : h->n_bclass[EDGE_BCLASS_FS16] + h->n_bclass[EDGE_BCLASS_FS16P] == h->n_cfg ? 8 : h->n_bclass[EDGE_BCLASS_FS8] == h->n_cfg ? 16
                            : h->n_bclass[EDGE_BCLASS_FS4] == h->n_cfg ? 32 : 0;
            const dim3 grid = uni ? dim3((unsigned)((h->slot_cap + 255) / 256), 1) : dim3(h->n_cfg, 12);
            hipLaunchKernelGGL(k_reduce_gpart, grid, dim3(256), 0, st, M, n_groups, layer_sets, G, counters, h->d_gpart.as<float>(),
                               sv.gbar, (long long)h->slot_cap, uni);
        } else if (n_groups > 1) {
            const int cls_only = h->n_bclass[EDGE_BCLASS_FS16] + h->n_bclass[EDGE_BCLASS_FS16P] == h->n_cfg ? EDGE_BCLASS_FS16
                                 : h->n_bclass[EDGE_BCLASS_FS8] == h->n_cfg ? EDGE_BCLASS_FS8
                                 : h->n_bclass[EDGE_BCLASS_FS4] == h->n_cfg ? EDGE_BCLASS_FS4 : -1;
            if (cls_only >= 0 && !h->active_mask && (layer_sets == 1 || n_gather == 0))
                hipLaunchKernelGGL(k_reduce_gbar_groups_uniform, dim3((unsigned)((h->slot_cap + 255) / 256)), dim3(256), 0, st, M,
                                   n_groups, counters, sv.gbar, (long long)h->slot_cap);
            else
                hipLaunchKernelGGL(k_reduce_gbar_groups, dim3(h->n_cfg, 12), dim3(256), 0, st, M, n_groups, layer_sets, G, counters, sv.gbar,
                                   (long long)h->slot_cap);
        }
        hipLaunchKernelGGL(k_finalize_forces, dim3((N + 3) / 4), dim3(256), 0, st, N, M, G, counters, sv.gbar,
                           (long long)h->slot_cap * fin_groups, h->units_per_ev, h->d_forces.as<float>(),
                           h->d_forces_std.as<float>());
    }
    hipLaunchKernelGGL(k_finalize_energy, dim3(h->n_cfg), dim3(256), 0, st, N, M, h->active_mask, G.cfg_start, Z, sv.e_atom,
                       h->units_per_ev, h->has_offset ? h->offset_per_z.as<double>() : (const double *)nullptr,
                       h->offset_const, h->d_energy.as<float>(), h->d_energy_std.as<float>(),
                       h->d_energy_models.as<float>(), h->d_energy64.as<double>(), h->d_e_atoms.as<float>(),
                       h->d_sat.as<unsigned>(), h->d_sat_out.as<unsigned>());
    P.end(st);
    VSSR_HIP(h, hipGetLastError());
    return VSSR_OK;
}

void painn_finalize(vssr_handle *h, const GraphView &G, uint32_t want, long long gbar_model_stride) {
    const int N = h->n_atoms, M = h->n_models;
    hipStream_t st = h->stream;
    if (want & VSSR_WANT_FORCES)
        hipLaunchKernelGGL(k_finalize_forces, dim3((N + 3) / 4), dim3(256), 0, st, N, M, G, h->d_counters.as<int>(), h->sv.gbar,
                           gbar_model_stride, h->units_per_ev, h->d_forces.as<float>(), h->d_forces_std.as<float>());
    hipLaunchKernelGGL(k_finalize_energy, dim3(h->n_cfg), dim3(256), 0, st, N, M, h->active_mask, G.cfg_start, h->d_Z.as<int>(),
                       h->sv.e_atom, h->units_per_ev, h->has_offset ? h->offset_per_z.as<double>() : (const double *)nullptr,
                       h->offset_const, h->d_energy.as<float>(), h->d_energy_std.as<float>(), h->d_energy_models.as<float>(),
                       h->d_energy64.as<double>(), h->d_e_atoms.as<float>(), h->d_sat.as<unsigned>(), h->d_sat_out.as<unsigned>());
}

int painn_stress(vssr_handle *h) {
    if (h->d_stress.ensure(sizeof(double) * 12 * (size_t)h->n_cfg)) return set_err(h, VSSR_E_DEVICE, "out of device memory (stress)");
    GraphView G{};
    G.n_atoms = h->n_atoms;
    G.n_cfg = h->n_cfg;
    G.cfg_start = h->d_cfg_start.as<int>();
    G.row_start = h->d_row_start.as<int>();
    G.edge = h->d_edge.as<float4>();
    const int fin_groups = h->gbar_mode == 2 ? 1 : painn_gbar_groups(h);
    double *out = h->d_stress.as<double>();
    hipLaunchKernelGGL(k_stress, dim3(h->n_cfg), dim3(256), 0, h->stream, h->n_models, G, h->d_counters.as<int>(), h->sv.gbar,
                       (long long)h->slot_cap * fin_groups, h->d_cell.as<double>(), h->units_per_ev, out, out + 6 * (size_t)h->n_cfg);
    VSSR_HIP(h, hipGetLastError());
    return VSSR_OK;
}

}
```

### surface-sampling_amd/csrc/painn_l0.hip

```cpp
#include "mfma16.h"

namespace vssr {

constexpr int KP = 24;
constexpr int TBLK = 4 * KP;

template <int NZ>
__global__ void __launch_bounds__(96)
k_l0_accum(GraphView G, const int *__restrict__ counters, float *__restrict__ T) {
    constexpr int nz = NZ;
    if (counters[2] || !G.act.atom(blockIdx.x)) return;
    const int i = blockIdx.x, comp = threadIdx.x / KP, kap = threadIdx.x % KP;
    float acc[NZ];
#pragma unroll
    for (int z = 0; z < NZ; ++z) acc[z] = 0.f;
    auto erec_c = [&](int idx) -> float4 {
#if defined(__HIP_DEVICE_COMPILE__)
        typedef const f32x4 __attribute__((address_space(4))) *cp;
        const f32x4 v = reinterpret_cast<cp>(reinterpret_cast<uintptr_t>(G.erec))[idx];
        return make_float4(v.x, v.y, v.z, v.w);
#else
        return G.erec[idx];
#endif
    };
    auto zslot_c = [&](int word) -> unsigned {
#if defined(__HIP_DEVICE_COMPILE__)
        typedef const unsigned __attribute__((address_space(4))) *cp;
        return reinterpret_cast<cp>(reinterpret_cast<uintptr_t>(G.zslot))[word];
#else
        return reinterpret_cast<const unsigned *>(G.zslot)[word];
#endif
    };
    const int e_begin = __builtin_amdgcn_readfirstlane(G.row_start[i]), e_end = __builtin_amdgcn_readfirstlane(G.row_start[i + 1]);
    for (int e = e_begin; e < e_end; e += 4) {
        float4 er[4];
        float r[4];
        int zi[4];
        const unsigned zw = zslot_c(e >> 2);
#pragma unroll
        for (int u = 0; u < 4; ++u) {
            er[u] = erec_c(e + u);
            r[u] = G.rho[(size_t)(e + u) * KP + kap];
            zi[u] = (zw >> (8 * u)) & 255;
        }
#pragma unroll
        for (int u = 0; u < 4; ++u) {
            const float uu = comp == 0 ? 1.f : comp == 1 ? er[u].x : comp == 2 ? er[u].y : er[u].z;
            const float val = r[u] * uu;
#pragma unroll
            for (int z = 0; z < NZ; ++z) acc[z] += (z == zi[u]) ? val : 0.f;
        }
    }
#pragma unroll
    for (int z = 0; z < NZ; ++z) T[((size_t)i * nz + z) * TBLK + comp * KP + kap] = acc[z];
}

constexpr int L0_TILE_U4 = 1024;

__global__ void __launch_bounds__(NTHREADS)
k_l0_fwd16(int N, int M, int nz, ActiveView av, const int *__restrict__ counters, const int *__restrict__ Z,
           const int *__restrict__ zlist, const ModelW *__restrict__ MW, const uint4 *__restrict__ A16, int n_embed,
           const float *__restrict__ T, float *__restrict__ s_msg, float *__restrict__ v_msg) {
    extern __shared__ __attribute__((aligned(16))) _Float16 ldsh[];
    if (counters[2]) return;
    const int K = 32 * nz, a0 = blockIdx.x * TA;
    if (!av.tile(min(a0, N - 1), min(a0 + TA - 1, N - 1))) return;
    const Planes Ts = make_planes(ldsh, TA, K), Tv = make_planes(ldsh + plane_halves(TA, K), 3 * TA, K);
    const LaneGeo L;
    SatTrack sat;
    const int lane = threadIdx.x & 63, r = lane & 15, g = lane >> 4;
    for (int t = threadIdx.x; t < TA * nz * 4 * 8; t += NTHREADS) {
        const int k4 = t & 7, comp = (t >> 3) & 3, z = (t >> 5) % nz, a = t / (32 * nz);
        float4 val = make_float4(0.f, 0.f, 0.f, 0.f);
        if (4 * k4 < KP)
            val = *reinterpret_cast<const float4 *>(T + ((size_t)min(a0 + a, N - 1) * nz + z) * TBLK + comp * KP + 4 * k4);
        if (comp == 0) store_split4<SAT_ANY>(Ts, a, 32 * z + 4 * k4, val, sat);
        else store_split4<SAT_ANY>(Tv, (comp - 1) * TA + a, 32 * z + 4 * k4, val, sat);
    }
    sat.commit(av, a0, N);
    __syncthreads();
    u32x4 bn[2][2];
    auto load_w = [&](int mm, int qq) {
        const uint4 *wb = A16 + (((size_t)mm * n_embed + zlist[qq]) * 2) * L0_TILE_U4 + (size_t)L.w * 128 + lane;
#pragma unroll
        for (int sec = 0; sec < 2; ++sec)
#pragma unroll
            for (int pc = 0; pc < 2; ++pc) bn[sec][pc] = gload4u(wb + sec * L0_TILE_U4 + pc * 64);
    };
    load_w(0, 0);
    for (int m = 0; m < M; ++m) {
        f32x4 acc[8];
#pragma unroll
        for (int t = 0; t < 8; ++t) acc[t] = (f32x4){0.f, 0.f, 0.f, 0.f};
#pragma unroll 1
        for (int q = 0; q < nz; ++q) {
            u32x4 b[2][2], a[8][2];
#pragma unroll
            for (int sec = 0; sec < 2; ++sec)
#pragma unroll
                for (int pc = 0; pc < 2; ++pc) b[sec][pc] = bn[sec][pc];
            {
                const int qn = q + 1 < nz ? q + 1 : 0, mn = q + 1 < nz ? m : m + 1;
                if (mn < M) load_w(mn, qn);
            }
#pragma unroll
            for (int t = 0; t < 8; ++t) {
                const Planes &P = t < 2 ? Ts : Tv;
                const int row = (t < 2 ? 16 * t : 16 * (t - 2)) + r;
                a[t][0] = *reinterpret_cast<const u32x4 *>(P.h + row * P.ld + 32 * q + 8 * g);
                a[t][1] = *reinterpret_cast<const u32x4 *>(P.l + row * P.ld + 32 * q + 8 * g);
            }
            __builtin_amdgcn_sched_barrier(0);
#pragma unroll
            for (int k = 0; k < 3; ++k)
#pragma unroll
                for (int t = 0; t < 8; ++t) {
                    acc[t] = mfma16(b[t < 2 ? 0 : 1][k == 0 ? 1 : 0], a[t][k == 1 ? 1 : 0], acc[t]);
                    __builtin_amdgcn_sched_barrier(0);
                }
        }
#pragma unroll
        for (int t = 0; t < 2; ++t) {
            const int a_ = a0 + L.row(t);
            if (a_ >= N) continue;
            const size_t gI = (size_t)m * N + a_;
            *reinterpret_cast<f32x4 *>(s_msg + gI * F + L.col0) = gload4f(MW[m].embed + (size_t)Z[a_] * F + L.col0) + acc[t];
#pragma unroll
            for (int x = 0; x < 3; ++x) *reinterpret_cast<f32x4 *>(v_msg + (gI * 3 + x) * F + L.col0) = acc[2 + 2 * x + t];
        }
    }
}

__global__ void __launch_bounds__(NTHREADS)
k_l0_q16(int N, int nz, ActiveView av, const int *__restrict__ counters, const int *__restrict__ zlist, const uint4 *__restrict__ At16,
         int n_embed, const float *__restrict__ sbar_msg, const float *__restrict__ vbar_msg,
         float *__restrict__ Q ) {
    extern __shared__ __attribute__((aligned(16))) _Float16 ldsh[];
    if (counters[2]) return;
    const int a0 = blockIdx.x * TA, m = blockIdx.y;
    if (!av.tile(min(a0, N - 1), min(a0 + TA - 1, N - 1))) return;
    const size_t mN = (size_t)m * N;
    const Planes Xs = make_planes(ldsh, TA, F), Xv = make_planes(ldsh + plane_halves(TA, F), 3 * TA, F);
    SatTrack sat;
    load_rows_split<TA>(Xs, 0, [&](int row) { return sbar_msg + (mN + min(a0 + row, N - 1)) * F; }, sat);
    load_rows_split<3 * TA>(Xv, 0, [&](int row) {
        int x = row / TA, a = min(a0 + (row % TA), N - 1);
        return vbar_msg + ((mN + a) * 3 + x) * F;
    }, sat);
    sat.commit(av, a0, N);
    __syncthreads();
    const int lane = threadIdx.x & 63, r = lane & 15, g = lane >> 4, w = threadIdx.x >> 6;
    for (int ct = w; ct < 2 * nz; ct += NW) {
        const int q = ct >> 1, hf = ct & 1;
        const uint4 *wb = At16 + (((size_t)m * n_embed + zlist[q]) * 2) * L0_TILE_U4 + (size_t)hf * 512 + lane;
        f32x4 acc[8];
#pragma unroll
        for (int t = 0; t < 8; ++t) acc[t] = (f32x4){0.f, 0.f, 0.f, 0.f};
        u32x4 bb[2][2][2];
        auto load_w = [&](int buf, int c) {
#pragma unroll
            for (int sec = 0; sec < 2; ++sec)
#pragma unroll
                for (int pc = 0; pc < 2; ++pc) bb[buf][sec][pc] = gload4u(wb + sec * L0_TILE_U4 + (c * 2 + pc) * 64);
        };
        load_w(0, 0);
#pragma unroll
        for (int c = 0; c < F / 32; ++c) {
            u32x4 (&b)[2][2] = bb[c & 1];
            u32x4 a[8][2];
            if (c + 1 < F / 32) load_w((c + 1) & 1, c + 1);
#pragma unroll
            for (int t = 0; t < 8; ++t) {
                const Planes &P = t < 2 ? Xs : Xv;
                const int row = (t < 2 ? 16 * t : 16 * (t - 2)) + r;
                a[t][0] = *reinterpret_cast<const u32x4 *>(P.h + row * P.ld + 32 * c + 8 * g);
                a[t][1] = *reinterpret_cast<const u32x4 *>(P.l + row * P.ld + 32 * c + 8 * g);
            }
            __builtin_amdgcn_sched_barrier(0);
#pragma unroll
            for (int k = 0; k < 3; ++k)
#pragma unroll
                for (int t = 0; t < 8; ++t) {
                    acc[t] = mfma16(a[t][k == 1 ? 1 : 0], b[t < 2 ? 0 : 1][k == 0 ? 1 : 0], acc[t]);
                    __builtin_amdgcn_sched_barrier(0);
                }
        }
        const int kap = 16 * hf + r;
        if (kap < KP) {
#pragma unroll
            for (int t = 0; t < 8; ++t) {
                const int comp = t < 2 ? 0 : 1 + (t - 2) / 2, tt = t < 2 ? t : (t - 2) & 1;
#pragma unroll
                for (int i = 0; i < 4; ++i) {
                    const int a_ = a0 + 16 * tt + 4 * g + i;
                    if (a_ < N) Q[((((size_t)m * N + a_) * nz + q) * 4 + comp) * KP + kap] = acc[t][i];
                }
            }
        }
    }
}

__global__ void __launch_bounds__(256)
k_l0_bwd(int N, int M, int nz, int first_write, int fresh_mfma, int excl_vol, float rc, GraphView G, const int *__restrict__ counters,
         const float *__restrict__ Q, float4 *__restrict__ gbar, long long gbar_group_stride, int n_groups) {
    extern __shared__ __attribute__((aligned(16))) float qs_all[];
    const int lane = threadIdx.x & 63, wave = threadIdx.x >> 6, sl = lane >> 2, kq = lane & 3;
    const int n = blockIdx.x * (blockDim.x >> 6) + wave;
    if (n >= N || counters[2] || !G.act.atom(n)) return;
    const int per_model = nz * TBLK;
    const bool fw = first_write || (fresh_mfma && G.chain_class[G.atom_cfg[n]] != EDGE_BCLASS_GATHER);
    float *qs = qs_all + (size_t)wave * M * per_model;
    for (int m = 0; m < M; ++m) {
        const float4 *src = reinterpret_cast<const float4 *>(Q + ((size_t)m * N + n) * per_model);
        for (int i = lane; i < per_model / 4; i += 64) reinterpret_cast<float4 *>(qs + m * per_model)[i] = src[i];
    }
    __builtin_amdgcn_fence(__ATOMIC_RELEASE, "wavefront");
    __builtin_amdgcn_wave_barrier();
    __builtin_amdgcn_fence(__ATOMIC_ACQUIRE, "wavefront");
    const int e0 = G.row_start[n], e1 = G.row_start[n + 1];
    for (int eb = e0; eb < e1; eb += 16) {
        const int e = min(eb + sl, e1 - 1);
        const bool live = eb + sl < e1;
        const float4 ed = G.edge[e];
        const float2 dd = G.dist2[e];
        const int zi = G.zslot[e];
        const int re = G.rev[e];
        float rho[6], drho[6], inv;
        bool valid;
        radial_quarter(ed, kq, rc, rho, drho, inv, valid);
        const float4 er = make_float4(ed.x * inv, ed.y * inv, ed.z * inv, 0.f);
        const bool real = live && zi < nz && re >= 0 && valid;
        const int zq = zi < nz ? zi : 0;
        for (int m = 0; m < M; ++m) {
            const float *q = qs + m * per_model + zq * TBLK + kq * 6;
            float qv[4][6];
#pragma unroll
            for (int cq = 0; cq < 4; ++cq)
#pragma unroll
                for (int k = 0; k < 3; ++k) {
                    const float2 t2 = reinterpret_cast<const float2 *>(q + cq * KP)[k];
                    qv[cq][2 * k] = t2.x; qv[cq][2 * k + 1] = t2.y;
                }
            float d0 = 0.f, dx = 0.f, dy = 0.f, dz = 0.f, bx = 0.f, by = 0.f, bz = 0.f;
#pragma unroll
            for (int k = 0; k < 6; ++k) {
                const float q0 = qv[0][k], qx = qv[1][k], qy = qv[2][k], qz = qv[3][k];
                d0 = fmaf(drho[k], q0, d0);
                dx = fmaf(drho[k], qx, dx); dy = fmaf(drho[k], qy, dy); dz = fmaf(drho[k], qz, dz);
                bx = fmaf(rho[k], qx, bx); by = fmaf(rho[k], qy, by); bz = fmaf(rho[k], qz, bz);
            }
            auto qsum = [](float x) {
                x += __builtin_bit_cast(float, __builtin_amdgcn_update_dpp(0, __builtin_bit_cast(int, x), 0xB1, 0xF, 0xF, true));
                x += __builtin_bit_cast(float, __builtin_amdgcn_update_dpp(0, __builtin_bit_cast(int, x), 0x4E, 0xF, 0xF, true));
                return x;
            };
            d0 = qsum(d0); dx = qsum(dx); dy = qsum(dy); dz = qsum(dz); bx = qsum(bx); by = qsum(by); bz = qsum(bz);
            if (real && kq == 0) {
                const float ux = -er.x, uy = -er.y, uz = -er.z;
                float db = d0 - (dx * ux + dy * uy + dz * uz);
                if (excl_vol) db += dd.y;
                const float invd = inv;
                const float dotu = fmaf(bz, uz, fmaf(by, uy, bx * ux));
                float g0 = fmaf(-db, ux, (bx - dotu * ux) * invd);
                float g1 = fmaf(-db, uy, (by - dotu * uy) * invd);
                float g2 = fmaf(-db, uz, (bz - dotu * uz) * invd);
                float4 *gb = gbar + (size_t)m * n_groups * gbar_group_stride;
                if (!fw) {
                    const float4 old = gb[re];
                    g0 += old.x; g1 += old.y; g2 += old.z;
                }
                gb[re] = make_float4(g0, g1, g2, 0.f);
            }
        }
    }
}

void l0_build_tables(const float *blob_embed, const float *W1, const float *b1, const float *W2, const float *b2,
                     const float *Wd, const float *bd, int n_embed, float *A ,
                     float *At ) {
    std::vector<float> h(F), phi(F3);
    for (int z = 0; z < n_embed; ++z) {
        const float *s = blob_embed + (size_t)z * F;
        for (int o = 0; o < F; ++o) {
            float acc = b1[o];
            for (int k = 0; k < F; ++k) acc = fmaf(W1[(size_t)o * F + k], s[k], acc);
            h[o] = acc / (1.f + expf(-acc));
        }
        for (int o = 0; o < F3; ++o) {
            float acc = b2[o];
            for (int k = 0; k < F; ++k) acc = fmaf(W2[(size_t)o * F + k], h[k], acc);
            phi[o] = acc;
        }
        for (int sec = 0; sec < 2; ++sec)
            for (int kap = 0; kap < KP; ++kap) {
                const int kq = kap / 6, ks = kap % 6;
                const int k = ks < 5 ? kq + 4 * ks : (kq == 0 ? 20 : 99);
                for (int f = 0; f < F; ++f) {
                    const int row = (sec + 1) * F + f;
                    const float w = k < 20 ? Wd[(size_t)row * 20 + k] : (k == 20 ? bd[row] : 0.f);
                    const float val = phi[row] * w;
                    A[(((size_t)z * 2 + sec) * KP + kap) * F + f] = val;
                    At[(((size_t)z * 2 + sec) * F + f) * KP + kap] = val;
                }
            }
    }
}

void l0_pack_tables(const float *A , int n_embed, unsigned *A16, unsigned *At16) {
    std::vector<float> fk((size_t)F * 32), kf((size_t)32 * F);
    for (int z = 0; z < n_embed; ++z)
        for (int sec = 0; sec < 2; ++sec) {
            std::fill(fk.begin(), fk.end(), 0.f);
            std::fill(kf.begin(), kf.end(), 0.f);
            for (int kap = 0; kap < KP; ++kap)
                for (int f = 0; f < F; ++f) {
                    const float v = A[(((size_t)z * 2 + sec) * KP + kap) * F + f];
                    fk[(size_t)f * 32 + kap] = v;
                    kf[(size_t)kap * F + f] = v;
                }
            const size_t o = ((size_t)z * 2 + sec) * L0_TILE_U4 * 4;
            pack_mfma_tiles16(fk.data(), F, 32, A16 + o);
            pack_mfma_tiles16(kf.data(), 32, F, At16 + o);
        }
}
size_t l0_packed_dwords(int n_embed) { return (size_t)n_embed * 2 * L0_TILE_U4 * 4; }

int l0_mfma_init(vssr_handle *h) {
    VSSR_HIP(h, hipFuncSetAttribute((const void *)k_l0_fwd16, hipFuncAttributeMaxDynamicSharedMemorySize, 160 * 1024));
    VSSR_HIP(h, hipFuncSetAttribute((const void *)k_l0_q16, hipFuncAttributeMaxDynamicSharedMemorySize, 160 * 1024));
    return VSSR_OK;
}

int l0_run_forward(vssr_handle *h, const GraphView &G, float *s_msg, float *v_msg) {
    const int N = h->n_atoms, M = h->n_models, nz = h->l0_nz;
    hipStream_t st = h->stream;
    if (h->d_l0T.ensure(sizeof(float) * (size_t)N * nz * TBLK) ||
        h->d_l0Q.ensure(sizeof(float) * (size_t)M * N * nz * TBLK))
        return set_err(h, VSSR_E_NOMEM, "layer-0 factorisation buffers: out of device memory");
    if (!h->l0T_by_geom) {
        const int *cnt = h->d_counters.as<int>();
        float *T = h->d_l0T.as<float>();
        switch (nz) {
            case 1: hipLaunchKernelGGL(k_l0_accum<1>, dim3(N), dim3(96), 0, st, G, cnt, T); break;
            case 2: hipLaunchKernelGGL(k_l0_accum<2>, dim3(N), dim3(96), 0, st, G, cnt, T); break;
            case 3: hipLaunchKernelGGL(k_l0_accum<3>, dim3(N), dim3(96), 0, st, G, cnt, T); break;
            case 4: hipLaunchKernelGGL(k_l0_accum<4>, dim3(N), dim3(96), 0, st, G, cnt, T); break;
            case 5: hipLaunchKernelGGL(k_l0_accum<5>, dim3(N), dim3(96), 0, st, G, cnt, T); break;
            case 6: hipLaunchKernelGGL(k_l0_accum<6>, dim3(N), dim3(96), 0, st, G, cnt, T); break;
            case 7: hipLaunchKernelGGL(k_l0_accum<7>, dim3(N), dim3(96), 0, st, G, cnt, T); break;
            default: hipLaunchKernelGGL(k_l0_accum<L0_MAX_SPECIES>, dim3(N), dim3(96), 0, st, G, cnt, T); break;
        }
    }
    const size_t lds_fwd = sizeof(_Float16) * (plane_halves(TA, 32 * nz) + plane_halves(3 * TA, 32 * nz));
    hipLaunchKernelGGL(k_l0_fwd16, dim3((N + TA - 1) / TA), dim3(NTHREADS), lds_fwd, st, N, M, nz, G.act, h->d_counters.as<int>(),
                       h->d_Z.as<int>(), h->d_zlist.as<int>(), h->model_table.as<ModelW>(), h->d_l0A.as<uint4>(), h->n_embed,
                       h->d_l0T.as<float>(), s_msg, v_msg);
    return VSSR_OK;
}

int l0_run_reverse(vssr_handle *h, const GraphView &G, int first_write, int fresh_mfma, const float *sbar_msg, const float *vbar_msg,
                   float4 *gbar, long long gbar_stride, int n_groups) {
    const int N = h->n_atoms, M = h->n_models, nz = h->l0_nz;
    hipStream_t st = h->stream;
    const size_t lds_q = sizeof(_Float16) * (plane_halves(TA, F) + plane_halves(3 * TA, F));
    hipLaunchKernelGGL(k_l0_q16, dim3((N + TA - 1) / TA, M), dim3(NTHREADS), lds_q, st, N, nz, G.act, h->d_counters.as<int>(),
                       h->d_zlist.as<int>(), h->d_l0At.as<uint4>(), h->n_embed, sbar_msg, vbar_msg, h->d_l0Q.as<float>());
    if (sizeof(float) * 4 * M * nz * TBLK > 48 * 1024)
        VSSR_HIP(h, hipFuncSetAttribute((const void *)k_l0_bwd, hipFuncAttributeMaxDynamicSharedMemorySize, 160 * 1024));
    hipLaunchKernelGGL(k_l0_bwd, dim3((N + 3) / 4), dim3(256), sizeof(float) * 4 * M * nz * TBLK, st, N, M, nz, first_write, fresh_mfma,
                       h->excl_vol, h->cutoff, G, h->d_counters.as<int>(), h->d_l0Q.as<float>(), gbar, gbar_stride, n_groups);
    return VSSR_OK;
}

}
```

### surface-sampling_amd/csrc/painn_node_mfma.hip

```cpp
#include "mfma16.h"

#ifdef PHASE_TIMING
__device__ unsigned long long g_phase[64];
#define PH_INIT unsigned long long ph_t = wall_clock64();
#define PH_RESET ph_t = wall_clock64();
#define PH(k) { const unsigned long long ph_n = wall_clock64(); if (threadIdx.x == 0) atomicAdd(&g_phase[k], ph_n - ph_t); ph_t = wall_clock64(); }
extern "C" int vssr_debug_phases(unsigned long long *out, int reset) {
    if (hipMemcpyFromSymbol(out, HIP_SYMBOL(g_phase), sizeof(unsigned long long) * 64) != hipSuccess) return -1;
    if (reset) { unsigned long long z[64] = {}; if (hipMemcpyToSymbol(HIP_SYMBOL(g_phase), z, sizeof(z)) != hipSuccess) return -1; }
    return 0;
}
#else
#define PH_INIT
#define PH_RESET
#define PH(k)
#endif

namespace vssr {

template <int NRT, int NCT>
struct GemmShape {
    static constexpr int NT = NRT * NCT, NACC = NT >= 3 ? 1 : 2;
};
template <int NRT, int NCT, int NPRE>
// ... 369 lines not shown
#ifndef UPD_SAVE_LATE
#define UPD_SAVE_LATE 1
#endif
constexpr int UPD_SAVE_UV = 0, UPD_SAVE_H3 = 12, UPD_SAVE_GATE = 14, UPD_SAVE_REGS = 18;
__device__ __forceinline__ f32x4 &save_slot(f32x4 *save, int m, int k) {
    return save[(((size_t)m * gridDim.x + blockIdx.x) * UPD_SAVE_REGS + k) * NTHREADS + threadIdx.x];
}
size_t update_save_bytes(int N, int M) { return sizeof(f32x4) * (size_t)M * ((N + TA - 1) / TA) * UPD_SAVE_REGS * NTHREADS; }

template <int TAIL>
__global__ void __launch_bounds__(NTHREADS) __attribute__((amdgpu_waves_per_eu(2, 2)))
k_update_fwd_mfma(int N, int l, ActiveView av, const ModelW *__restrict__ MW, const float *__restrict__ s_msg,
                  const float *__restrict__ v_msg, float *__restrict__ s_out, float *__restrict__ v_out,
                  float *__restrict__ phi_next, f32x4 *__restrict__ save) {
    extern __shared__ __attribute__((aligned(16))) _Float16 ldsh[];
    constexpr bool NOV = TAIL == 2;
    const int m = blockIdx.y, a0 = blockIdx.x * TA;
    if (!av.tile(min(a0, N - 1), min(a0 + TA - 1, N - 1))) return;
    const LaneGeo L;
    SatTrack sat;
    const LayerW &W = MW[m].layer[l];
    const size_t mN = (size_t)m * N;
    const Planes vt = make_planes(ldsh, 3 * TA, F), xs = make_planes(ldsh + CF_XS, TA, F);
    const Planes nr = make_planes(ldsh, TA, F), as_ = make_planes(ldsh + plane_halves(TA, F), TA, F);
    constexpr int PF = 1;
    float4 keep_v[3 * TA * (F / 4) / NTHREADS], keep_s[TA * (F / 4) / NTHREADS];
    PH_INIT
    const uint4 *wUV[2] = {WTILE(U, L.w, F), WTILE(V, L.w, F)};
    const uint4 *wW3a[1] = {WTILE(W3, L.w, 2 * F)};
    const uint4 *wW3b[1] = {WTILE(W3, L.w, 2 * F) + (F / 32) * 2 * 64};
    const uint4 *wW4[3] = {WTILE(W4, L.w, F), WTILE(W4, NW + L.w, F), WTILE(W4, 2 * NW + L.w, F)};
    WPre<6, 2, 1> pUV;
    WPre<2, 1, 1> pW3a;
    rows_request<3 * TA>([&](int row) {
        int x = row / TA, a = min(a0 + (row % TA), N - 1);
        return v_msg + ((mN + a) * 3 + x) * F;
    }, keep_v);
    rows_request<TA>([&](int row) { return s_msg + (mN + min(a0 + row, N - 1)) * F; }, keep_s);
    __builtin_amdgcn_sched_barrier(0);
    gemm16_preload(wUV, pUV);
    gemm16_preload(wW3a, pW3a);
    rows_store_split<3 * TA>(vt, 0, keep_v, sat);
    rows_store_split<TA>(xs, 0, keep_s, sat);
    __syncthreads();
    PH(0)
    f32x4 uv[6][2];
    zero_acc(uv);
    gemm16<F, 6, 2, PF, 1>(vt, wUV, uv, &pUV);
    PH(1)
    f32x4 h3[2][1];
    zero_acc(h3);
    gemm16<F, 2, 1, PF, 1>(xs, wW3a, h3, &pW3a);
    WPre<2, 1, 2> pW3b;
    gemm16_preload(wW3b, pW3b);
    PH(2)
    __syncthreads();
    PH(3)
    f32x4 inner[2];
#pragma unroll
    for (int t = 0; t < 2; ++t) {
        f32x4 nv;
#pragma unroll
        for (int i = 0; i < 4; ++i) {
            float n2 = 0.f, in = 0.f;
#pragma unroll
            for (int x = 0; x < 3; ++x) {
                const float vv = uv[2 * x + t][1][i];
                n2 += fmaf(vv, vv, 1e-15f);
                in = fmaf(uv[2 * x + t][0][i], vv, in);
            }
            inner[t][i] = in;
            nv[i] = sqrtf(n2);
        }
        store_split4(nr, L.row(t), L.col0, nv, sat);
    }
    __syncthreads();
    PH(4)
    WPre<2, 3, 1> pW4;
    WPre<2, 2, 1> pW4n;
    const uint4 *wW4n[2] = {wW4[1], wW4[2]};
    {
        const f32x4 b = gload4f(W.b3 + L.col0);
        __builtin_amdgcn_sched_barrier(0);
        gemm16<F, 2, 1, PF, 2>(nr, wW3b, h3, &pW3b);
        if constexpr (NOV) gemm16_preload(wW4n, pW4n); else gemm16_preload(wW4, pW4);
#pragma unroll
        for (int t = 0; t < 2; ++t) {
            f32x4 sw = h3[t][0] + b;
            h3[t][0] = sw;
#pragma unroll
            for (int i = 0; i < 4; ++i) sw[i] = swish(sw[i]);
            store_split4(as_, L.row(t), L.col0, sw, sat);
        }
    }
    PH(5)
    __syncthreads();
    PH(6)
    f32x4 gate[2][3];
    zero_acc(gate);
    const uint4 *wW1n[1] = {nullptr}, *wW2n[3] = {nullptr, nullptr, nullptr};
    WPre<2, 1, 2> pW1n;
    {
        f32x4 b4[3];
#pragma unroll
        for (int c = 0; c < 3; ++c) b4[c] = gload4f(W.b4 + c * F + L.col0);
        __builtin_amdgcn_sched_barrier(0);
        if constexpr (NOV) {
            f32x4 g2[2][2];
            zero_acc(g2);
            gemm16<F, 2, 2, PF, 1>(as_, wW4n, g2, &pW4n);
#pragma unroll
            for (int t = 0; t < 2; ++t) { gate[t][1] = g2[t][0]; gate[t][2] = g2[t][1]; }
        } else {
            gemm16<F, 2, 3, PF, 1>(as_, wW4, gate, &pW4);
        }
        if constexpr (TAIL == 1) {
            const LayerW &Wn = MW[m].layer[l + 1];
            wW1n[0] = Wn.qW1 + (size_t)L.w * 4 * F;
#pragma unroll
            for (int c = 0; c < 3; ++c) wW2n[c] = Wn.qW2 + (size_t)(c * NW + L.w) * 4 * F;
            gemm16_preload(wW1n, pW1n);
        }
#pragma unroll
        for (int c = 0; c < 3; ++c) {
#pragma unroll
            for (int t = 0; t < 2; ++t) gate[t][c] += b4[c];
        }
    }
    auto save_all = [&]() {
        if (!save) return;
#pragma unroll
        for (int j = 0; j < 6; ++j)
#pragma unroll
            for (int c = 0; c < 2; ++c) save_slot(save, m, UPD_SAVE_UV + 2 * j + c) = uv[j][c];
#pragma unroll
        for (int t = 0; t < 2; ++t) {
            save_slot(save, m, UPD_SAVE_H3 + t) = h3[t][0];
#pragma unroll
            for (int c = 0; c < 2; ++c) save_slot(save, m, UPD_SAVE_GATE + 2 * t + c) = gate[t][c];
        }
    };
#if UPD_SAVE_LATE == 0
    save_all();
#endif
    PH(7)
    __syncthreads();
    PH(8)
    float *T = reinterpret_cast<float *>(ldsh);
#pragma unroll
    for (int t = 0; t < 2; ++t) {
        const int row = L.row(t);
        f32x4 ds;
#pragma unroll
        for (int i = 0; i < 4; ++i) ds[i] = fmaf(gate[t][1][i], inner[t][i], gate[t][2][i]);
        *reinterpret_cast<f32x4 *>(T + row * FT + L.col0) = ds;
        if constexpr (!NOV) {
#pragma unroll
            for (int x = 0; x < 3; ++x) *reinterpret_cast<f32x4 *>(T + (TA * (1 + x) + row) * FT + L.col0) = gate[t][0] * uv[2 * x + t][0];
        }
    }
    __syncthreads();
    auto gofs = [&](int row, int col) -> size_t {
        const int q = row / TA, a = min(a0 + row % TA, N - 1);
        return q == 0 ? (mN + a) * F + col : ((mN + a) * 3 + (q - 1)) * F + col;
    };
    PH(9)
    const Planes xo = make_planes(ldsh + CF_LDS_HALVES, TA, F);
    auto put = [&](int row, int col, const float4 &d, const float4 &r) {
        const float4 o = make_float4(r.x + d.x, r.y + d.y, r.z + d.z, r.w + d.w);
        if (TAIL == 1 && row < TA) store_split4<SAT_COOP>(xo, row, col, o, sat);
        if (a0 + row % TA >= N) return;
        if (row >= TA && !v_out) return;
        *reinterpret_cast<float4 *>((row < TA ? s_out : v_out) + gofs(row, col)) = o;
    };
    {
        constexpr int NS = TA * (F / 4) / NTHREADS, NV = 3 * TA * (F / 4) / NTHREADS;
#pragma unroll
        for (int it = 0; it < (NOV ? NS : NS + NV); ++it) {
            const int idx = threadIdx.x + it * NTHREADS, row = idx >> 5, c4 = idx & 31;
            put(row, 4 * c4, *reinterpret_cast<const float4 *>(T + row * FT + 4 * c4), it < NS ? keep_s[it < NS ? it : 0] : keep_v[it < NS ? 0 : it - NS]);
        }
    }
    PH(10)
    if constexpr (TAIL == 1) {
        const LayerW &Wn = MW[m].layer[l + 1];
        const Planes hn = make_planes(ldsh, TA, F);
        __syncthreads();
        WPre<2, 3, 1> pW2n;
        {
            f32x4 acc[2][1];
            zero_acc(acc);
            const f32x4 b = gload4f(Wn.b1 + L.col0);
            __builtin_amdgcn_sched_barrier(0);
            gemm16<F, 2, 1, 1, 2>(xo, wW1n, acc, &pW1n);
            gemm16_preload(wW2n, pW2n);
#pragma unroll
            for (int t = 0; t < 2; ++t) {
                f32x4 hv = acc[t][0] + b;
#pragma unroll
                for (int i = 0; i < 4; ++i) hv[i] = swish(hv[i]);
                store_split4(hn, L.row(t), L.col0, hv, sat);
            }
        }
        __syncthreads();
        f32x4 acc[2][3];
        zero_acc(acc);
        f32x4 b2[3];
#pragma unroll
        for (int c = 0; c < 3; ++c) b2[c] = gload4f(Wn.b2 + c * F + L.col0);
        __builtin_amdgcn_sched_barrier(0);
        gemm16<F, 2, 3, 1, 1>(hn, wW2n, acc, &pW2n);
#pragma unroll
        for (int c = 0; c < 3; ++c) {
            const f32x4 b = b2[c];
#pragma unroll
            for (int t = 0; t < 2; ++t) {
                const int a = a0 + L.row(t);
                if (a < N) *reinterpret_cast<f32x4 *>(phi_next + (mN + a) * F3 + c * F + L.col0) = acc[t][c] + b;
            }
        }
        PH(11)
    }
#if UPD_SAVE_LATE
    save_all();
#endif
    sat.commit(av, a0, N);
}

constexpr int RH = 64;
template <int RT, bool WANT_SBAR, class Sat>
__device__ __forceinline__ void readout_head(const ModelW &W, const Planes &xs, const Planes &hp, float *red, const LaneGeo &L,
                                             int a0, int N, size_t mN, const float *__restrict__ e_excl,
                                             float *__restrict__ e_atom, f32x4 (&sb)[RT], Sat &sat) {
    constexpr int NCW = RH / 16;
    constexpr int TA = 16 * RT;
    const int lane = threadIdx.x & 63;
    if (L.w < NCW) {
        f32x4 acc[RT][1];
        zero_acc(acc);
        const uint4 *wp[1] = {W.qW5 + (size_t)L.w * 4 * F};
        const f32x4 b = gload4f(W.b5 + L.col0), w6 = gload4f(W.w6 + L.col0);
        __builtin_amdgcn_sched_barrier(0);
        gemm16<F, RT, 1>(xs, wp, acc);
#pragma unroll
        for (int t = 0; t < RT; ++t) {
            const f32x4 hval = acc[t][0] + b;
            f32x4 hb;
            float es = 0.f;
#pragma unroll
            for (int i = 0; i < 4; ++i) {
                es = fmaf(w6[i], swish(hval[i]), es);
                hb[i] = w6[i] * dswish(hval[i]);
            }
            if (WANT_SBAR) store_split4(hp, L.row(t), L.col0, hb, sat);
            es = xrow_sum_f32(es);
            if (lane < 16) red[L.w * TA + L.row(t)] = es;
        }
    }
    __syncthreads();
    if (threadIdx.x < TA) {
        const int atom = a0 + threadIdx.x;
        if (atom < N) {
            float e = gload1f(W.b6);
#pragma unroll
            for (int k = 0; k < NCW; ++k) e += red[k * TA + threadIdx.x];
            if (e_excl) e += e_excl[atom];
            e_atom[mN + atom] = e;
        }
    }
    if (WANT_SBAR) {
        f32x4 acc[RT][1];
        zero_acc(acc);
        const uint4 *wp[1] = {W.qW5t + (size_t)L.w * 4 * RH};
        gemm16<RH, RT, 1>(hp, wp, acc);
#pragma unroll
        for (int t = 0; t < RT; ++t) sb[t] = acc[t][0];
    }
}

__global__ void __launch_bounds__(NTHREADS)
k_readout_mfma(int N, ActiveView av, const ModelW *__restrict__ MW, const float *__restrict__ s, const float *__restrict__ e_excl,
               float *__restrict__ e_atom) {
    extern __shared__ __attribute__((aligned(16))) _Float16 ldsh[];
    const int m = blockIdx.y, a0 = blockIdx.x * TA;
    if (!av.tile(min(a0, N - 1), min(a0 + TA - 1, N - 1))) return;
    const LaneGeo L;
    SatTrack sat;
    const size_t mN = (size_t)m * N;
    const Planes xs = make_planes(ldsh, TA, F), hp = make_planes(ldsh + plane_halves(TA, F), TA, RH);
    float *red = reinterpret_cast<float *>(ldsh + plane_halves(TA, F) + plane_halves(TA, RH));
    load_rows_split<TA>(xs, 0, [&](int row) { return s + (mN + min(a0 + row, N - 1)) * F; }, sat);
    __syncthreads();
    f32x4 sb[2];
    readout_head<2, false>(MW[m], xs, hp, red, L, a0, N, mN, e_excl, e_atom, sb, sat);
    sat.commit(av, a0, N);
}

template <int MODE, int RT, bool SAVED = false>
__global__ void __launch_bounds__(NTHREADS) __attribute__((amdgpu_waves_per_eu(RT == 1 ? 4 : 2, RT == 1 ? 4 : 2)))
k_update_bwd_mfma(int N, int l, int vbar_is_zero, ActiveView av, const ModelW *__restrict__ MW, const float *__restrict__ s_msg,
                  const float *__restrict__ v_msg, const float *__restrict__ sbar_src, const float *__restrict__ vbar,
                  const float *__restrict__ s_next, const float *__restrict__ phibar, const float *__restrict__ e_excl,
                  float *__restrict__ e_atom, float *__restrict__ sbar_msg, float *__restrict__ vbar_msg,
                  const f32x4 *__restrict__ save) {
    static_assert(!SAVED || RT == 2, "the saved layout is that of the 32-atom forward kernel");
    extern __shared__ __attribute__((aligned(16))) _Float16 ldsh[];
    constexpr int TA = 16 * RT, OFF_VT = UpdLds<RT>::OFF_VT, OFF_AS = UpdLds<RT>::OFF_AS, UPD_LDS_HALVES = UpdLds<RT>::HALVES;
    const int m = blockIdx.y, a0 = blockIdx.x * TA;
    if (!av.tile(min(a0, N - 1), min(a0 + TA - 1, N - 1))) return;
    const LaneGeo L;
    constexpr int BPF = MODE == 0 ? 0 : UPD_PF;
    SatNone unwatched;
    const LayerW &W = MW[m].layer[l];
    const size_t mN = (size_t)m * N;
    PH_INIT
    f32x4 sb[RT];
    if (MODE != 1) {
#pragma unroll
        for (int t = 0; t < RT; ++t) sb[t] = gload4f(sbar_src + (mN + min(a0 + L.row(t), N - 1)) * F + L.col0);
    }
    float *VB = reinterpret_cast<float *>(ldsh + UPD_LDS_HALVES);
    if (MODE == 1) vbar_is_zero = 1;
    if (!vbar_is_zero) {
        constexpr int NIT = 3 * TA * (F / 4) / NTHREADS;
        float4 vv[NIT];
#pragma unroll
        for (int it = 0; it < NIT; ++it) {
            const int idx = threadIdx.x + it * NTHREADS, row = idx >> 5, c4 = idx & 31;
            vv[it] = *reinterpret_cast<const float4 *>(vbar + ((mN + min(a0 + row % TA, N - 1)) * 3 + row / TA) * F + 4 * c4);
        }
#pragma unroll
        for (int it = 0; it < NIT; ++it) {
            const int idx = threadIdx.x + it * NTHREADS, row = idx >> 5, c4 = idx & 31;
            *reinterpret_cast<float4 *>(VB + row * FT + 4 * c4) = vv[it];
        }
    }
    UpdRegs<RT> R;
    auto load_saved = [&]() {
        const f32x4 *sv = save + (((size_t)m * gridDim.x + blockIdx.x) * UPD_SAVE_REGS) * NTHREADS + threadIdx.x;
#pragma unroll
        for (int j = 0; j < 3 * RT; ++j)
#pragma unroll
            for (int c = 0; c < 2; ++c) R.uv[j][c] = gload4f(reinterpret_cast<const float *>(sv + (size_t)(UPD_SAVE_UV + 2 * j + c) * NTHREADS));
#pragma unroll
        for (int t = 0; t < RT; ++t) {
            R.h3[t] = gload4f(reinterpret_cast<const float *>(sv + (size_t)(UPD_SAVE_H3 + t) * NTHREADS));
#pragma unroll
            for (int c = 0; c < 2; ++c) R.gate[t][c] = gload4f(reinterpret_cast<const float *>(sv + (size_t)(UPD_SAVE_GATE + 2 * t + c) * NTHREADS));
        }
    };
    if (!SAVED) load_update_s<RT>(ldsh, s_msg, mN, a0, N, unwatched);
    else load_saved();
    if (MODE == 0) {
        load_update_v<RT>(ldsh, v_msg, mN, a0, N, unwatched);
        __syncthreads();
    } else if (MODE == 1) {
        if (!SAVED) load_update_v<RT>(ldsh, v_msg, mN, a0, N, unwatched);
        const Planes xs = make_planes(ldsh + OFF_AS, TA, F);
        const Planes hp = make_planes(ldsh + UPD_LDS_HALVES, TA, RH);
        float *red = reinterpret_cast<float *>(ldsh + UPD_LDS_HALVES + plane_halves(TA, RH));
        {
            SatTrack satc;
            load_rows_split<TA>(xs, 0, [&](int row) { return s_next + (mN + min(a0 + row, N - 1)) * F; }, satc);
            satc.commit(av, a0, N);
        }
        __syncthreads();
        PH(40)
        {
            SatTrack sate;
            readout_head<RT, true>(MW[m], xs, hp, red, L, a0, N, mN, e_excl, e_atom, sb, sate);
            sate.commit(av, a0, N);
        }
        PH(41)
    } else {
        const LayerW &Wn = MW[m].layer[l + 1];
        const Planes xs = make_planes(ldsh + OFF_AS, TA, F), pb = make_planes(ldsh + OFF_VT, TA, F3);
        load_rows_split<TA>(xs, 0, [&](int row) { return s_next + (mN + min(a0 + row, N - 1)) * F; }, unwatched);
        {
            SatTrack satc;
#pragma unroll
            for (int c = 0; c < 3; ++c)
                load_rows_split<TA>(pb, c * F, [&](int row) { return phibar + (mN + min(a0 + row, N - 1)) * F3 + c * F; }, satc);
            satc.commit(av, a0, N);
        }
        __syncthreads();
        PH(42)
        f32x4 h1[RT][1], a1[RT][1];
        zero_acc(h1);
        zero_acc(a1);
        const f32x4 b1n = gload4f(Wn.b1 + L.col0);
        __builtin_amdgcn_sched_barrier(0);
        {
            const uint4 *wp[1] = {Wn.qW1 + (size_t)L.w * 4 * F};
            gemm16<F, RT, 1, BPF>(xs, wp, h1);
            const uint4 *wq[1] = {Wn.qW2t + (size_t)L.w * 4 * F3};
            gemm16<F3, RT, 1, BPF>(pb, wq, a1);
        }
        PH(43)
        __syncthreads();
        if (!SAVED) load_update_v<RT>(ldsh, v_msg, mN, a0, N, unwatched);
        PH(44)
        {
            const f32x4 b = b1n;
            SatTrack sate;
#pragma unroll
            for (int t = 0; t < RT; ++t) {
                f32x4 hv;
#pragma unroll
                for (int i = 0; i < 4; ++i) hv[i] = a1[t][0][i] * dswish(h1[t][0][i] + b[i]);
                store_split4(xs, L.row(t), L.col0, hv, sate);
            }
            sate.commit(av, a0, N);
        }
        __syncthreads();
        f32x4 acc[RT][1];
        zero_acc(acc);
        const uint4 *wp[1] = {Wn.qW1t + (size_t)L.w * 4 * F};
        gemm16<F, RT, 1, BPF>(xs, wp, acc);
#pragma unroll
        for (int t = 0; t < RT; ++t) sb[t] += acc[t][0];
        PH(45)
    }
    PH(16)
    if constexpr (!SAVED) {
        update_forward<RT, 16, BPF>(W, ldsh, L, R, unwatched);
    } else {
#pragma unroll
        for (int t = 0; t < RT; ++t)
#pragma unroll
            for (int i = 0; i < 4; ++i) {
                float in = 0.f;
#pragma unroll
                for (int x = 0; x < 3; ++x) in = fmaf(R.uv[RT * x + t][0][i], R.uv[RT * x + t][1][i], in);
                R.inner[t][i] = in;
            }
        __syncthreads();
    }
    PH_RESET
    const Planes qb = make_planes(ldsh + OFF_VT, TA, F3);
    SatTrack sat;
#pragma unroll
    for (int t = 0; t < RT; ++t) {
        const int row = L.row(t);
        f32x4 abar_vv = {0.f, 0.f, 0.f, 0.f};
        if (!vbar_is_zero) {
#pragma unroll
            for (int x = 0; x < 3; ++x) {
                const f32x4 vb = *reinterpret_cast<const f32x4 *>(VB + (x * TA + row) * FT + L.col0);
#pragma unroll
                for (int i = 0; i < 4; ++i) abar_vv[i] = fmaf(vb[i], R.uv[RT * x + t][0][i], abar_vv[i]);
            }
        }
        store_split4(qb, row, L.col0, abar_vv, sat);
        store_split4(qb, row, F + L.col0, sb[t] * R.inner[t], sat);
        store_split4(qb, row, 2 * F + L.col0, sb[t], sat);
    }
    sat.commit(av, a0, N);
    sat = SatTrack();
    PH(23)
    __syncthreads();
    PH(24)
    const Planes hb = make_planes(ldsh + OFF_AS, TA, F);
    {
        f32x4 acc[RT][1];
        zero_acc(acc);
        const uint4 *wp[1] = {WTILE(W4t, L.w, F3)};
        gemm16<F3, RT, 1, BPF>(qb, wp, acc);
#pragma unroll
        for (int t = 0; t < RT; ++t) {
            f32x4 hv;
#pragma unroll
            for (int i = 0; i < 4; ++i) hv[i] = acc[t][0][i] * dswish(R.h3[t][i]);
            store_split4(hb, L.row(t), L.col0, hv, sat);
        }
        sat.commit(av, a0, N);
        sat = SatTrack();
    }
    PH(25)
    __syncthreads();
    PH(26)
    f32x4 hbar[RT][2];
    zero_acc(hbar);
    {
        const uint4 *wp[2] = {WTILE(W3t, L.w, F), WTILE(W3t, NW + L.w, F)};
        gemm16<F, RT, 2, BPF>(hb, wp, hbar);
    }
    PH(27)
    __syncthreads();
    PH(28)
    const Planes ab = make_planes(ldsh, 3 * TA, 2 * F);
#pragma unroll
    for (int t = 0; t < RT; ++t) {
        const int row = L.row(t);
        f32x4 sc, sa;
#pragma unroll
        for (int i = 0; i < 4; ++i) {
            float n2 = 0.f;
#pragma unroll
            for (int x = 0; x < 3; ++x) {
                const float vv = R.uv[RT * x + t][1][i];
                n2 += fmaf(vv, vv, 1e-15f);
            }
            sc[i] = hbar[t][1][i] / sqrtf(n2);
            sa[i] = sb[t][i] * R.gate[t][1][i];
        }
#pragma unroll
        for (int x = 0; x < 3; ++x) {
            f32x4 vbo = {0.f, 0.f, 0.f, 0.f};
            if (!vbar_is_zero) vbo = *reinterpret_cast<const f32x4 *>(VB + (x * TA + row) * FT + L.col0);
            f32x4 ub, vb2;
#pragma unroll
            for (int i = 0; i < 4; ++i) {
                const float u = R.uv[RT * x + t][0][i], v = R.uv[RT * x + t][1][i];
                ub[i] = fmaf(vbo[i], R.gate[t][0][i], sa[i] * v);
                vb2[i] = fmaf(sa[i], u, sc[i] * v);
            }
            store_split4(ab, x * TA + row, L.col0, ub, sat);
            store_split4(ab, x * TA + row, F + L.col0, vb2, sat);
        }
    }
    sat.commit(av, a0, N);
    PH(29)
    __syncthreads();
    PH(30)
    f32x4 out[3 * RT][1];
    zero_acc(out);
    {
        const uint4 *wp[1] = {WTILE(UVt, L.w, 2 * F)};
        gemm16<2 * F, 3 * RT, 1, BPF>(ab, wp, out);
    }
    PH(31)
    __syncthreads();
    PH(32)
    float *T = reinterpret_cast<float *>(ldsh);
#pragma unroll
    for (int t = 0; t < RT; ++t) {
        const int row = L.row(t);
        *reinterpret_cast<f32x4 *>(T + row * FT + L.col0) = sb[t] + hbar[t][0];
#pragma unroll
        for (int x = 0; x < 3; ++x) *reinterpret_cast<f32x4 *>(T + (TA * (1 + x) + row) * FT + L.col0) = out[RT * x + t][0];
    }
    __syncthreads();
    stage_rows<4 * TA>(T, [&](int row, int col, const float4 &d) {
        const int q = row / TA, a = a0 + row % TA;
        if (a >= N) return;
        if (q == 0) {
            *reinterpret_cast<float4 *>(sbar_msg + (mN + a) * F + col) = d;
        } else {
            const size_t off = ((mN + a) * 3 + (q - 1)) * F + col;
            float4 r = make_float4(0.f, 0.f, 0.f, 0.f);
            if (!vbar_is_zero) r = *reinterpret_cast<const float4 *>(VB + (row - TA) * FT + col);
            *reinterpret_cast<float4 *>(vbar_msg + off) = make_float4(r.x + d.x, r.y + d.y, r.z + d.z, r.w + d.w);
        }
    });
    PH(33)
}

void pack_mfma_tiles16(const float *Wsrc, int rows, int K, unsigned *dst) {
    auto split2 = [](float x, unsigned (&p)[2]) {
        const _Float16 h = (_Float16)x;
        const _Float16 l = (_Float16)(x - (float)h);
        unsigned short hb, lb;
        memcpy(&hb, &h, 2);
        memcpy(&lb, &l, 2);
        p[0] = hb; p[1] = lb;
    };
    const int ntile = rows / 16, nq = K / 32;
    for (int tile = 0; tile < ntile; ++tile)
        for (int q = 0; q < nq; ++q)
            for (int lane = 0; lane < 64; ++lane)
                for (int j = 0; j < 4; ++j) {
                    const size_t row = (size_t)tile * 16 + (lane & 15);
                    const int k = 32 * q + 8 * (lane >> 4) + 2 * j;
                    unsigned p0[2], p1[2];
                    split2(Wsrc[row * K + k], p0);
                    split2(Wsrc[row * K + k + 1], p1);
                    for (int pc = 0; pc < 2; ++pc)
                        dst[((((size_t)tile * nq + q) * 2 + pc) * 64 + lane) * 4 + j] = p0[pc] | (p1[pc] << 16);
                }
}

size_t node_mfma_lds_bytes(int which) {
    switch (which) {
        case 0: return sizeof(_Float16) * 2 * plane_halves(TA, F);
        case 1: return sizeof(_Float16) * (plane_halves(TA, F) + plane_halves(TA, F3));
        case 4: return sizeof(_Float16) * (plane_halves(TA, F) + plane_halves(TA, RH)) + sizeof(float) * (RH / 16) * TA;
        case 6: return 96 * 1024;
        default: return sizeof(_Float16) * UpdLds<2>::HALVES + sizeof(float) * 3 * TA * FT;
    }
}
static_assert(sizeof(_Float16) * plane_halves(16, RH) + sizeof(float) * (RH / 16) * 16 <= sizeof(float) * 3 * 16 * FT,
              "readout scratch fits the vbar region");

static_assert(sizeof(_Float16) * (CF_LDS_HALVES + plane_halves(TA, F)) <= 96 * 1024, "update fwd LDS request");

bool readout_mfma_supported(int hidden) { return hidden == RH; }

int node_mfma_init(vssr_handle *h) {
    VSSR_HIP(h, hipFuncSetAttribute((const void *)k_msg_mlp_mfma<2, 0>, hipFuncAttributeMaxDynamicSharedMemorySize, 96 * 1024));
    VSSR_HIP(h, hipFuncSetAttribute((const void *)k_msg_mlp_bwd_mfma, hipFuncAttributeMaxDynamicSharedMemorySize,
                                    (int)node_mfma_lds_bytes(1)));
    VSSR_HIP(h, hipFuncSetAttribute((const void *)k_update_fwd_mfma<0>, hipFuncAttributeMaxDynamicSharedMemorySize,
                                    (int)node_mfma_lds_bytes(6)));
    VSSR_HIP(h, hipFuncSetAttribute((const void *)k_update_fwd_mfma<1>, hipFuncAttributeMaxDynamicSharedMemorySize,
                                    (int)node_mfma_lds_bytes(6)));
    VSSR_HIP(h, hipFuncSetAttribute((const void *)k_update_fwd_mfma<2>, hipFuncAttributeMaxDynamicSharedMemorySize,
                                    (int)node_mfma_lds_bytes(6)));
#define SET_UPD(MODE)                                                                                                     \
    VSSR_HIP(h, hipFuncSetAttribute((const void *)k_update_bwd_mfma<MODE, 2>, hipFuncAttributeMaxDynamicSharedMemorySize, \
                                    (int)node_mfma_lds_bytes(3)));
    SET_UPD(0) SET_UPD(1) SET_UPD(2)
#undef SET_UPD
    VSSR_HIP(h, hipFuncSetAttribute((const void *)k_update_bwd_mfma<1, 2, true>, hipFuncAttributeMaxDynamicSharedMemorySize,
                                    (int)node_mfma_lds_bytes(3)));
    VSSR_HIP(h, hipFuncSetAttribute((const void *)k_update_bwd_mfma<2, 2, true>, hipFuncAttributeMaxDynamicSharedMemorySize,
                                    (int)node_mfma_lds_bytes(3)));
    VSSR_HIP(h, hipFuncSetAttribute((const void *)k_readout_mfma, hipFuncAttributeMaxDynamicSharedMemorySize,
                                    (int)node_mfma_lds_bytes(4)));
    return VSSR_OK;
}

void launch_msg_mlp_mfma(hipStream_t st, int N, int M, int l, const ActiveView &av, const ModelW *MW, const float *s_in,
                         float *phi) {
    hipLaunchKernelGGL((k_msg_mlp_mfma<2, 0>), dim3((N + TA - 1) / TA, M), dim3(NTHREADS), node_mfma_lds_bytes(0), st, N, l, av, MW,
                       s_in, phi);
}
void launch_msg_mlp_bwd_mfma(hipStream_t st, int N, int M, int l, const ActiveView &av, const ModelW *MW, const float *s_in,
                             const float *phibar, const float *sbar_msg, float *sbar_in) {
    hipLaunchKernelGGL(k_msg_mlp_bwd_mfma, dim3((N + TA - 1) / TA, M), dim3(NTHREADS), node_mfma_lds_bytes(1), st, N, l, av, MW,
                       s_in, phibar, sbar_msg, sbar_in);
}
void launch_update_fwd_mfma(hipStream_t st, int N, int M, int l, const ActiveView &av, const ModelW *MW, const float *s_msg,
                            const float *v_msg, float *s_out, float *v_out, float *phi_next, void *save) {
    f32x4 *sv = reinterpret_cast<f32x4 *>(save);
    if (phi_next)
        hipLaunchKernelGGL(k_update_fwd_mfma<1>, dim3((N + TA - 1) / TA, M), dim3(NTHREADS), node_mfma_lds_bytes(6), st, N, l,
                           av, MW, s_msg, v_msg, s_out, v_out, phi_next, sv);
    else if (!v_out && !sv)
        hipLaunchKernelGGL(k_update_fwd_mfma<2>, dim3((N + TA - 1) / TA, M), dim3(NTHREADS), node_mfma_lds_bytes(6), st, N, l,
                           av, MW, s_msg, v_msg, s_out, v_out, phi_next, sv);
    else
        hipLaunchKernelGGL(k_update_fwd_mfma<0>, dim3((N + TA - 1) / TA, M), dim3(NTHREADS), node_mfma_lds_bytes(6), st, N, l,
                           av, MW, s_msg, v_msg, s_out, v_out, phi_next, sv);
}
void launch_readout_mfma(hipStream_t st, int N, int M, const ActiveView &av, const ModelW *MW, const float *s,
                         const float *e_excl, float *e_atom) {
    hipLaunchKernelGGL(k_readout_mfma, dim3((N + TA - 1) / TA, M), dim3(NTHREADS), node_mfma_lds_bytes(4), st, N, av, MW, s,
                       e_excl, e_atom);
}
void launch_update_bwd_mfma(hipStream_t st, int N, int M, int l, int mode, int vbar_is_zero, const ActiveView &av, const ModelW *MW,
                            const float *s_msg, const float *v_msg, const float *sbar_src, const float *vbar,
                            const float *s_next, const float *phibar, const float *e_excl, float *e_atom,
                            float *sbar_msg, float *vbar_msg, const void *save) {
    const f32x4 *sv = reinterpret_cast<const f32x4 *>(save);
    if (mode == 1) vbar_is_zero = 1;
#if defined(UPD_BWD_RT) && UPD_BWD_RT == 1
    if (!sv && mode != 0) {
        const dim3 grid1((N + 15) / 16, M), blk1(NTHREADS);
        const size_t lds1 = sizeof(_Float16) * UpdLds<1>::HALVES + sizeof(float) * 3 * 16 * FT;
        static bool once = [] {
            (void)hipFuncSetAttribute((const void *)k_update_bwd_mfma<1, 1, false>, hipFuncAttributeMaxDynamicSharedMemorySize, 80 * 1024);
            (void)hipFuncSetAttribute((const void *)k_update_bwd_mfma<2, 1, false>, hipFuncAttributeMaxDynamicSharedMemorySize, 80 * 1024);
            return true;
        }();
        (void)once;
        if (mode == 1)
            hipLaunchKernelGGL((k_update_bwd_mfma<1, 1, false>), grid1, blk1, lds1, st, N, l, vbar_is_zero, av, MW, s_msg, v_msg, sbar_src,
                               vbar, s_next, phibar, e_excl, e_atom, sbar_msg, vbar_msg, sv);
        else
            hipLaunchKernelGGL((k_update_bwd_mfma<2, 1, false>), grid1, blk1, lds1, st, N, l, vbar_is_zero, av, MW, s_msg, v_msg, sbar_src,
                               vbar, s_next, phibar, e_excl, e_atom, sbar_msg, vbar_msg, sv);
        return;
    }
#endif
    const dim3 grid((N + TA - 1) / TA, M), blk(NTHREADS);
    const size_t lds = node_mfma_lds_bytes(3);
#define LAUNCH_UPD(MODE, SAVED)                                                                                             \
    hipLaunchKernelGGL((k_update_bwd_mfma<MODE, 2, SAVED>), grid, blk, lds, st, N, l, vbar_is_zero, av, MW, s_msg, v_msg, sbar_src, \
                       vbar, s_next, phibar, e_excl, e_atom, sbar_msg, vbar_msg, sv)
    if (mode == 1) { if (sv) LAUNCH_UPD(1, true); else LAUNCH_UPD(1, false); }
    else if (mode == 2) { if (sv) LAUNCH_UPD(2, true); else LAUNCH_UPD(2, false); }
    else LAUNCH_UPD(0, false);
#undef LAUNCH_UPD
}

}
```

### surface-sampling_amd/csrc/vssr_internal.h

```cpp
#pragma once

#include <hip/hip_runtime.h>

#include <cstdint>
#include <cstdio>
#include <cstdlib>
#include <cstring>
#include <memory>
#include <string>
#include <utility>
#include <vector>

#include "../../include/vssr_eval.h"

namespace vssr {

constexpr int F = 128;
constexpr int F3 = 3 * F;
constexpr int MAX_LAYERS = 4;
constexpr int MAX_MODELS = 8;
constexpr int RB_MAX = 24;
constexpr int NODE_TILE = 8;
constexpr int L0_MAX_SPECIES = 8;

struct LayerW {
    const float *W1, *W1t, *b1;
    const float *W2, *W2t, *b2;
    const float *Wd, *bd;
    const float *U, *Ut, *V, *Vt;
    const float *W3, *W3t, *b3;
    const float *W4, *W4t, *b4;
    const uint4 *qW1, *qW2, *qU, *qV, *qW3, *qW4, *qW1t, *qW2t, *qW4t, *qW3t, *qUVt;
    const uint4 *wd16;
};
struct ModelW {
    const float *embed;
    LayerW layer[MAX_LAYERS];
    const float *W5, *W5t, *b5, *w6, *b6;
    const uint4 *qW5, *qW5t;
};

struct ActiveView {
    const unsigned char *mask;
    const int *atom_cfg;
    unsigned *sat = nullptr;
    __device__ __forceinline__ bool chain(int c) const { return !mask || mask[c]; }
    __device__ __forceinline__ bool atom(int i) const { return !mask || mask[atom_cfg[i]]; }
    __device__ __forceinline__ bool tile(int a0, int a1) const {
        if (!mask) return true;
        for (int c = atom_cfg[a0], c1 = atom_cfg[a1]; c <= c1; ++c)
            if (mask[c]) return true;
        return false;
    }
};

struct GraphView {
    int n_atoms;
    int n_cfg;
    const int *atom_cfg;
    const int *cfg_start;
    const int *row_start;
    const int *deg;
    const float4 *edge;
    const int *rev;
    const float4 *erec;
    const float *rho;
    const uint4 *rho16;
    const uint4 *drho16;
    const unsigned char *zslot;
    const float2 *dist2;
    const int4 *bundle;
    const unsigned char *chain_class;
    ActiveView act;
};

#if defined(__HIPCC__)
__device__ __forceinline__ int wave_incl_scan_i32(int x) {
    x += __builtin_amdgcn_update_dpp(0, x, 0x111, 0xF, 0xF, true);
    x += __builtin_amdgcn_update_dpp(0, x, 0x112, 0xF, 0xF, true);
    x += __builtin_amdgcn_update_dpp(0, x, 0x114, 0xF, 0xF, true);
    x += __builtin_amdgcn_update_dpp(0, x, 0x118, 0xF, 0xF, true);
    x += __builtin_amdgcn_update_dpp(0, x, 0x142, 0xA, 0xF, false);
    x += __builtin_amdgcn_update_dpp(0, x, 0x143, 0xC, 0xF, false);
    return x;
}
__device__ __forceinline__ float xrow_sum_f32(float x) {
    const unsigned u = __float_as_uint(x);
    const auto r32 = __builtin_amdgcn_permlane32_swap(u, u, false, false);
    const float y = __uint_as_float(r32[0]) + __uint_as_float(r32[1]);
    const unsigned v = __float_as_uint(y);
    const auto r16 = __builtin_amdgcn_permlane16_swap(v, v, false, false);
    return __uint_as_float(r16[0]) + __uint_as_float(r16[1]);
}
__device__ __forceinline__ float wave_sum_f32(float x) {
    x += __builtin_bit_cast(float, __builtin_amdgcn_update_dpp(0, __builtin_bit_cast(int, x), 0xB1, 0xF, 0xF, true));
    x += __builtin_bit_cast(float, __builtin_amdgcn_update_dpp(0, __builtin_bit_cast(int, x), 0x4E, 0xF, 0xF, true));
    x += __builtin_bit_cast(float, __builtin_amdgcn_update_dpp(0, __builtin_bit_cast(int, x), 0x124, 0xF, 0xF, true));
    x += __builtin_bit_cast(float, __builtin_amdgcn_update_dpp(0, __builtin_bit_cast(int, x), 0x128, 0xF, 0xF, true));
    const unsigned u = __float_as_uint(x);
    const auto r32 = __builtin_amdgcn_permlane32_swap(u, u, false, false);
    const float y = __uint_as_float(r32[0]) + __uint_as_float(r32[1]);
    const unsigned v = __float_as_uint(y);
    const auto r16 = __builtin_amdgcn_permlane16_swap(v, v, false, false);
    return __uint_as_float(r16[0]) + __uint_as_float(r16[1]);
}
#endif

#if defined(__HIPCC__)
__device__ __forceinline__ void radial_quarter(const float4 &ed, int kq, float rc, float (&r)[6], float (&dr)[6], float &inv, bool &valid) {
    const float alpha = 3.14159265358979323846f / rc;
    valid = __float_as_int(ed.w) >= 0;
    const float d2 = fmaf(ed.z, ed.z, fmaf(ed.y, ed.y, ed.x * ed.x));
    const float d = valid ? sqrtf(d2) : 1.f;
    inv = valid ? 1.f / d : 0.f;
    float s1, c1;
    sincosf(alpha * d, &s1, &c1);
    const bool inside = valid && d < rc;
    const float fc = inside ? 0.5f * (c1 + 1.f) : 0.f;
    const float dfc = inside ? -0.5f * alpha * s1 : 0.f;
    const float s2 = 2.f * s1 * c1, c2 = fmaf(c1, c1, -s1 * s1);
    const float s3 = fmaf(s2, c1, c2 * s1), c3 = fmaf(c2, c1, -s2 * s1);
    const float s4 = 2.f * s2 * c2, c4 = fmaf(c2, c2, -s2 * s2);
    float sn = kq == 0 ? s1 : kq == 1 ? s2 : kq == 2 ? s3 : s4;
    float cn = kq == 0 ? c1 : kq == 1 ? c2 : kq == 2 ? c3 : c4;
    float nf = (float)(kq + 1);
#pragma unroll
    for (int ks = 0; ks < 5; ++ks) {
        const float rb = sn * inv;
        r[ks] = rb * fc;
        dr[ks] = fmaf(nf * alpha * cn * inv - rb * inv, fc, rb * dfc);
        const float sn2 = fmaf(sn, c4, cn * s4), cn2 = fmaf(cn, c4, -sn * s4);
        sn = sn2; cn = cn2; nf += 4.f;
    }
    r[5] = fc;
    dr[5] = dfc;
}
#endif

struct StateView {
    int n_atoms;
    int n_models;
    float *s_in[MAX_LAYERS + 1];
    float *v_in[MAX_LAYERS + 1];
    float *phi[MAX_LAYERS];
    float *s_msg[MAX_LAYERS];
    float *v_msg[MAX_LAYERS];
    float *e_atom;
    const float *e_excl;
    float *sbar;
    float *vbar;
    float *sbar_msg;
    float *sbar_msg_l0;
    float *vbar_msg;
    float *phibar;
    float4 *gbar;
};

struct DevBuf {
    void *p = nullptr;
    size_t bytes = 0;
    DevBuf() = default;
    DevBuf(const DevBuf &) = delete;
    DevBuf &operator=(const DevBuf &) = delete;
    ~DevBuf() { release(); }
    int ensure(size_t need) {
        if (need <= bytes) return 0;
        release();
        size_t want = need + need / 4 + 256;
        if (hipMalloc(&p, want) != hipSuccess) return -1;
        bytes = want;
        return 0;
    }
    void release() {
        if (p) (void)hipFree(p);
        p = nullptr;
        bytes = 0;
    }
    void swap(DevBuf &o) { std::swap(p, o.p); std::swap(bytes, o.bytes); }
    template <class T>
    T *as() const { return reinterpret_cast<T *>(p); }
};

struct OwnedStream {
    hipStream_t s = nullptr;
    OwnedStream() = default;
    OwnedStream(const OwnedStream &) = delete;
    OwnedStream &operator=(const OwnedStream &) = delete;
    ~OwnedStream() { if (s) (void)hipStreamDestroy(s); }
    operator hipStream_t() const { return s; }
};
struct PinnedInts {
    int *p = nullptr;
    PinnedInts() = default;
    PinnedInts(const PinnedInts &) = delete;
    PinnedInts &operator=(const PinnedInts &) = delete;
    ~PinnedInts() { if (p) (void)hipHostFree(p); }
    operator int *() const { return p; }
};

enum KernelClass {
    KC_NBR = 0,
    KC_EMBED,
    KC_MSG_MLP,
    KC_EDGE_FWD,
    KC_UPDATE_FWD,
    KC_READOUT,
    KC_UPDATE_BWD,
    KC_EDGE_BWD,
    KC_MSG_MLP_BWD,
    KC_FINALIZE,
    KC_ANALYTIC,
    KC_L0_FWD,
    KC_L0_BWD,
    KC_COUNT
};
extern const char *const kKernelClassNames[KC_COUNT];

struct Profiler {
    bool enabled = false;
    struct Rec { int kc; hipEvent_t a, b; };
    std::vector<Rec> pending;
    std::vector<hipEvent_t> pool;
    int64_t launches[KC_COUNT] = {0};
    double total_ms[KC_COUNT] = {0};
    hipEvent_t get_event();
    void begin(int kc, hipStream_t s);
    void end(hipStream_t s);
    void collect();
    void reset();
    Profiler() = default;
    Profiler(const Profiler &) = delete;
    Profiler &operator=(const Profiler &) = delete;
    ~Profiler();
};

struct GmmFit {
    int cov_type = 0;
    int init = 0;
    int max_iter = 100, n_init = 1;
    double tol = 1e-3, reg_covar = 1e-6;
    uint64_t seed = 0;
    bool device_ready = false, fitted = false;
    int64_t n = 0, cap = 0;
    DevBuf rows;
    double *x() const { return rows.as<double>(); }
    std::vector<double> i_means, i_weights, i_prec;
    std::vector<int> i_labels;
    bool has_means = false, has_weights = false, has_prec = false, has_labels = false;
    DevBuf resp, labels, lbpart, status, flags;
    DevBuf part_s, part_q, part_n, nk, means, avg_x2, w, cov, part_cov, chol_w, chol_y, centers, assign_part;
    DevBuf b_w, b_means, b_cov, b_P, b_c, b_kc, b_mask;
};

struct Cluster {
    int n_components = 0, whiten = 1, d_clu = 3, d_pad = 3;
    bool pca_done = false;
    int64_t n_pts = 0;
    DevBuf mean, denom, part_sum, part_cov, cov, evec, eval, comp, comp_t, ev, ratio, jac, xr;
    DevBuf pts;
    DevBuf cen[2], siz[2], cid[2];
    DevBuf nn, flag, blk, rec, counters;
};

enum class Kind : int {
    NONE = 0,
    PAINN = 1,
    TERSOFF = 2,
    EAM = 3,
    SW = 4,
    GMM = 5,
    GMM_FIT = 6,
    CLUSTER = 7,
    PAIR = 8,
    COUNT
};
constexpr unsigned kind_bit(Kind k) { return 1u << (int)k; }
constexpr unsigned KINDS_EVAL = kind_bit(Kind::PAINN) | kind_bit(Kind::TERSOFF) | kind_bit(Kind::EAM) | kind_bit(Kind::SW) |
                                kind_bit(Kind::PAIR);

}

struct vssr_handle {
    vssr::Kind kind = vssr::Kind::NONE;
    vssr_eam_grid eam_grid = {0, 0, 0.0, 0.0, 0.0};
    int eam_nel = 0, eam_fs = 0;
    int device = 0;
    vssr::OwnedStream stream;
    std::string err;
    vssr::Profiler prof;

    int edge_impl = 1;
    int max_cfg_atoms = 0;
    vssr::DevBuf d_chain_class, d_class_list;
    int n_class[5] = {0, 0, 0, 0, 0}, max_class_atoms[5] = {0, 0, 0, 0, 0};
    int n_bclass[5] = {0, 0, 0, 0, 0}, max_bclass_atoms[5] = {0, 0, 0, 0, 0};
    int fs16_max_atoms = -1, fs8_max_atoms = -1, fs4_max_atoms = -1;
    int max_images = 0;

    int n_models = 0, n_rbf = 20, num_conv = 3, n_embed = 100, readout_hidden = 64;
    int feat_dim = vssr::F;
    bool painn_general = false;
    float cutoff = 5.f;
    int excl_vol = 1, excl_power = 12;
    float excl_sigma = 1.5f;
    double units_per_ev = 1.0;
    bool has_offset = false;
    double offset_const = 0.0;

    vssr::DevBuf weights;
    vssr::DevBuf wd16;
    vssr::DevBuf node16;
    vssr::DevBuf model_table;
    vssr::DevBuf offset_per_z;

    int n_types = 0;
    double pot_cutoff = 0;
    vssr::DevBuf pot_params;

    bool batch_valid = false, ran = false;
    int n_cfg = 0, n_atoms = 0;
    std::vector<int> h_n_atoms, h_cfg_start;
    vssr::DevBuf d_pos, d_wpos, d_wrap, d_Z, d_atom_cfg, d_cfg_start, d_cell, d_invcell, d_nimg, d_pbc;
    vssr::DevBuf d_deg, d_row_start, d_edge, d_edge_S, d_rev, d_counters, d_tile_sums;
    vssr::DevBuf d_erec, d_rho, d_dist, d_rho16, d_drho16, d_zslot, d_bundle, d_excl;
    vssr::DevBuf d_bundle_sub;
    int bwd_multi_pass = 1;
    int fwd_mpass_fs8 = 1;
    int sub_chunk_fwd = 0, sub_chunk_bwd = 0;
    vssr::DevBuf d_bundle_subb;
    int fwd_two_pass = 16;
    vssr::DevBuf d_hits;
    int l0_enabled = 1, l0_nz = 0;
    bool l0_used = false;
    vssr::DevBuf d_l0A, d_l0At;
    vssr::DevBuf d_zmap, d_zlist;
    vssr::DevBuf d_l0T, d_l0Q;
    vssr::DevBuf d_opt_state, d_opt_vec, d_bfgs_q, d_bfgs_b, d_fixed, d_relax_steps, d_relax_conv, d_active;
    const unsigned char *active_mask = nullptr;
    int relax_regrows = 0;
    long long relax_lockstep = 0;
    int relax_compactions = 0;
    vssr::DevBuf d_cmp;
    vssr::DevBuf d_cm;
    long long relax_chain_evals = 0;
    int traj_interval = 0, traj_records = 0, traj_B = 0, traj_N = 0;
    vssr::DevBuf d_traj_pos, d_traj_f, d_traj_e, d_traj_n;
    bool graph_partial = false;
    bool l0T_by_geom = false;
    int64_t zero_entry_cap = -1;
    const void *zero_entry_tab[2] = {nullptr, nullptr};
    int cap_per_atom = 64;
    int cm_cap_per_atom = 0;
    bool cap_tight = false;
    uint32_t last_want = 0;
    int64_t slot_cap = 0;
    vssr::PinnedInts h_counters;

    vssr::DevBuf d_state;
    vssr::StateView sv;
    vssr::DevBuf d_gbar;
    vssr::DevBuf d_upd_save;
    int gbar_mode = 2;
    vssr::DevBuf d_gpart;
    int debug_keep = 0;
    int upd_save = 0;
    vssr::DevBuf d_energy, d_energy_std, d_energy_models, d_forces, d_forces_std, d_e_atoms;
    vssr::DevBuf d_energy64;
    vssr::DevBuf d_pot_e, d_pot_ea, d_pot_f;
    vssr::DevBuf d_sat, d_sat_out;
    std::vector<unsigned> h_sat;
    bool h_sat_valid = false;
    vssr::DevBuf d_stress;

    int gmm_K = 0, gmm_D = 0, gmm_Dp = 0;
    double gmm_log2pi = 0.0;
    vssr::DevBuf d_gmm_P;
    vssr::DevBuf d_gmm_c;
    vssr::DevBuf d_gmm_kc;
    vssr::DevBuf d_gmm_mask;
    vssr::DevBuf d_gmm_x, d_gmm_lp, d_gmm_nll, d_gmm_sys, d_gmm_start;
    std::unique_ptr<vssr::GmmFit> fit;
    std::unique_ptr<vssr::Cluster> clu;
};

namespace vssr {

int set_err(vssr_handle *h, int code, const char *fmt, ...);
#define VSSR_HIP(h, expr)                                                                    \
    do {                                                                                     \
        hipError_t _e = (expr);                                                              \
        if (_e != hipSuccess)                                                                \
            return vssr::set_err(h, VSSR_E_DEVICE, "%s failed: %s (%s:%d)", #expr,          \
                                 hipGetErrorString(_e), __FILE__, __LINE__);                 \
    } while (0)

int check_kind(vssr_handle *h, unsigned served, const char *func);
int device_in_range(vssr_handle *h, int device);
int open_device(vssr_handle *h, int device);
void publish_create_error(const vssr_handle *h);
template <class Init>
int create_handle(Kind kind, int device, vssr_handle **out, Init init, bool range_check = true) {
    vssr_handle *h = new vssr_handle();
    h->kind = kind;
    int rc = range_check ? device_in_range(h, device) : VSSR_OK;
    if (!rc) rc = open_device(h, device);
    if (!rc) rc = init(h);
    if (rc) {
        publish_create_error(h);
        vssr_destroy(h);
        return rc;
    }
    *out = h;
    return VSSR_OK;
}
int run_any(vssr_handle *h, uint32_t want);
int sync_and_check(vssr_handle *h);
int grow_slot_cap(vssr_handle *h);

int build_neighbors(vssr_handle *h, double cutoff);
int painn_alloc_state(vssr_handle *h);
int painn_run(vssr_handle *h, uint32_t want);
int painn_stress(vssr_handle *h);
int painn_alloc_results(vssr_handle *h);
void painn_finalize(vssr_handle *h, const GraphView &G, uint32_t want, long long gbar_model_stride);
int painn_gen_upload(vssr_handle *h, const vssr_painn_config *cfg);
int painn_gen_run(vssr_handle *h, uint32_t want);
int tersoff_run(vssr_handle *h, uint32_t want);
int eam_run(vssr_handle *h, uint32_t want);
int sw_run(vssr_handle *h, uint32_t want);
int pair_run(vssr_handle *h, uint32_t want);
int gmm_upload(vssr_handle *g, const double *means, const double *prec_chol, const double *weights);
int gmm_score_f64(vssr_handle *g, hipStream_t st, int64_t n, const double *x_dev);
int gmm_score_f32(vssr_handle *g, hipStream_t st, int64_t n, const float *x_dev);
int gmm_mean_rows(vssr_handle *g, hipStream_t st, int B, const int *start, const float *emb);
int gmm_reduce(vssr_handle *g, hipStream_t st, int B, const int *start, int order);
int gmm_fit_check_config(const vssr_gmm_fit_config *cfg);
int gmm_fit_append_host(vssr_handle *h, int64_t n_rows, const double *x);
int gmm_fit_append_f32(vssr_handle *h, hipStream_t st, int64_t n_rows, const float *emb_dev);
int gmm_fit_append_f64p(vssr_handle *h, hipStream_t st, int64_t n_rows, const double *x_dev);
int gmm_fit_set_init(vssr_handle *h, const double *means, const double *weights, const double *precisions, const int32_t *labels);
int gmm_fit_run(vssr_handle *h, vssr_gmm_fit_result *res);
int gmm_fit_params(vssr_handle *h, double *weights, double *means, double *covariances, double *prec_chol);
int gmm_fit_copy_scorer(vssr_handle *h, vssr_handle *g);
int gmm_fit_centered_cov(vssr_handle *h, hipStream_t st, const double *X, int n, int D, int Dp, const double *mean, const double *denom,
                         DevBuf &part, double *cov);
int cluster_pca(vssr_handle *h, vssr_cluster_pca_result *res);
int cluster_pca_params(vssr_handle *h, double *mean, double *components, double *explained_variance, double *ratio);
int cluster_projected(vssr_handle *h, int64_t first, int64_t n_rows, double *xr);
int cluster_set_points(vssr_handle *h, int64_t n, const double *pts);
int cluster_linkage(vssr_handle *h, double *Z, int32_t *n_rounds);
int cluster_pad_dims(int d);
int tersoff_stress(vssr_handle *h);
int eam_stress(vssr_handle *h);
int sw_stress(vssr_handle *h);
int pair_stress(vssr_handle *h);
struct Evaluator {
    bool f64;
    int (*run)(vssr_handle *h, uint32_t want);
    int (*stress)(vssr_handle *h);
    double (*cutoff)(const vssr_handle *h);
};
const Evaluator &evaluator(const vssr_handle *h);
inline bool is_analytic(const vssr_handle *h) { return evaluator(h).f64; }
void eam_build_spline(const double *f, int n, double delta, double *spl );
int relax_fire(vssr_handle *h, const vssr_fire_params &p, const uint8_t *fixed_host, uint32_t want);
int relax_bfgs(vssr_handle *h, const vssr_bfgs_params &p, const uint8_t *fixed_host, uint32_t want);
int relax_begin(vssr_handle *h, const uint8_t *fixed_host, int steps_ints_per_chain, const uint8_t *&fixed);
int relax_regrow(vssr_handle *h, int cap, long long &it, int window);
int relax_cg(vssr_handle *h, const vssr_cg_params *cp, const uint8_t *fixed_host, uint32_t want);
bool chain_min_supported(const vssr_handle *h);
int chain_min_cg(vssr_handle *h, const vssr_cg_params *cp, const uint8_t *fixed_host, uint32_t want);
int node_mfma_init(vssr_handle *h);
void launch_msg_mlp_mfma(hipStream_t st, int N, int M, int l, const ActiveView &av, const ModelW *MW, const float *s_in,
                         float *phi);
void launch_msg_mlp_bwd_mfma(hipStream_t st, int N, int M, int l, const ActiveView &av, const ModelW *MW, const float *s_in,
                             const float *phibar, const float *sbar_msg, float *sbar_in);
void launch_update_fwd_mfma(hipStream_t st, int N, int M, int l, const ActiveView &av, const ModelW *MW, const float *s_msg,
                            const float *v_msg, float *s_out, float *v_out, float *phi_next, void *save);
size_t update_save_bytes(int N, int M);
bool readout_mfma_supported(int hidden);
void launch_readout_mfma(hipStream_t st, int N, int M, const ActiveView &av, const ModelW *MW, const float *s, const float *e_excl,
                         float *e_atom);
void launch_update_bwd_mfma(hipStream_t st, int N, int M, int l, int mode, int vbar_is_zero, const ActiveView &av, const ModelW *MW,
                            const float *s_msg, const float *v_msg, const float *sbar_src, const float *vbar,
                            const float *s_next, const float *phibar, const float *e_excl, float *e_atom,
                            float *sbar_msg, float *vbar_msg, const void *save);
void pack_mfma_tiles16(const float *Wsrc, int rows, int K, unsigned *dst );
void build_wd16(const float *Wd, const float *bd, unsigned *dst );
void l0_build_tables(const float *blob_embed, const float *W1, const float *b1, const float *W2, const float *b2,
                     const float *Wd, const float *bd, int n_embed, float *A, float *At);
void l0_pack_tables(const float *A, int n_embed, unsigned *A16, unsigned *At16);
size_t l0_packed_dwords(int n_embed);
int l0_mfma_init(vssr_handle *h);
int l0_run_forward(vssr_handle *h, const GraphView &G, float *s_msg, float *v_msg);
int l0_run_reverse(vssr_handle *h, const GraphView &G, int first_write, int fresh_mfma, const float *sbar_msg, const float *vbar_msg,
                   float4 *gbar, long long gbar_stride, int n_groups);
int edge_mfma_init(vssr_handle *h);
enum { EDGE_CLASS_FS16 = 0, EDGE_CLASS_FS16M = 1, EDGE_CLASS_FS8 = 2, EDGE_CLASS_FS4 = 3, EDGE_CLASS_GATHER = 4, EDGE_CLASSES = 5,
       EDGE_MFMA_CLASSES = 4 };
enum { EDGE_BCLASS_FS16 = 0, EDGE_BCLASS_FS8 = 1, EDGE_BCLASS_FS4 = 2, EDGE_BCLASS_FS16P = 3, EDGE_BCLASS_GATHER = 4, EDGE_BCLASSES = 5,
       EDGE_MFMA_BCLASSES = 4 };
__host__ __device__ constexpr int edge_bclass_slices(int c) { return (c == EDGE_BCLASS_FS16 || c == EDGE_BCLASS_FS16P) ? 8 : c == EDGE_BCLASS_FS8 ? 16 : c == EDGE_BCLASS_FS4 ? 32 : 1; }
int edge_bclass_of(int n_atoms);
int edge_class_of(int n_atoms);
constexpr int SUB_MAX_PASSES = 4;
__host__ __device__ constexpr int sub_chunk_max(int width) { return width == 16 ? 400 : 784; }
__host__ __device__ constexpr int sub_chunk_max_bwd() { return 550; }
__host__ __device__ constexpr int sub_passes(int n_atoms, int chunk_max) { return (n_atoms + chunk_max - 1) / chunk_max; }
__host__ __device__ constexpr int sub_chunk(int n_atoms, int chunk_max) { return (n_atoms + sub_passes(n_atoms, chunk_max) - 1) / sub_passes(n_atoms, chunk_max); }
int edge_class_groups(int cls);
void launch_edge_bwd_mfma(hipStream_t st, int cls, int N, const int *list, int n_list, int M, int l, int layer_first, int max_atoms,
                          const ModelW *MW, const GraphView &G, const int *counters, int zero_slot,
                          const float *v_in, const float *phi, const float *sbar_msg, const float *vbar_msg,
                          float *phibar, float *vbar_in, float *gbar, long long gbar_stride, int n_groups, int group_off, int rec,
                          const int4 *bundle_sub, int sub_chunk);
void launch_edge_fwd_mfma(hipStream_t st, int cls, int N, const int *list, int n_list, int M, int l, int max_atoms, const ModelW *MW,
                          const GraphView &G, const int *counters, int zero_slot, const float *s_in, const float *v_in,
                          const float *phi, float *s_msg, float *v_msg, const int4 *bundle_sub, int sub_width, int sub_chunk);

}
```

Before: 24640 evaluations/s.

## Fuse layer-0 Q projection into the layer-0 update backward kernel

Adds a MODE 3 tail to the update backward kernel. At layer 0 it splits the adjoints straight into LDS planes and runs the Q-tile MFMA projection there. This removes the separate k_l0_q16 launch and the global write and re-read of sbar_msg/vbar_msg for layer 0. Those adjoints are now produced only on demand through a deferred recompute path used for debug readback, and the fused tile loop adds work and register pressure to the update kernel.

```diff
diff --git a/surface-sampling_amd/csrc/api_batch.hip b/surface-sampling_amd/csrc/api_batch.hip
--- a/surface-sampling_amd/csrc/api_batch.hip
+++ b/surface-sampling_amd/csrc/api_batch.hip
@@ -573,8 +573,13 @@
         src = sv.v_in[l + 1]; per_atom = F3;
     }
     else if (nm == "e_atom") { src = sv.e_atom; per_atom = 1; }
-    else if (nm == "sbar_msg0") { src = sv.sbar_msg_l0; per_atom = F; }
-    else if (nm == "vbar_msg0") { src = sv.vbar_msg; per_atom = F3; }
+    else if (nm == "sbar_msg0" || nm == "vbar_msg0") {
+        if (!(h->last_want & VSSR_WANT_FORCES))
+            return set_err(h, VSSR_E_STATE, "%s is not materialised (the last evaluation ran without forces: no reverse pass)", name);
+        if ((rc = painn_materialise_l0_adjoints(h))) return rc;
+        if (nm == "sbar_msg0") { src = sv.sbar_msg_l0; per_atom = F; }
+        else { src = sv.vbar_msg; per_atom = F3; }
+    }
     else return set_err(h, VSSR_E_BADARG, "unknown intermediate '%s'", name);
     size_t n = N * per_atom;
     *n_out = (int64_t)n;
diff --git a/surface-sampling_amd/csrc/api_painn.hip b/surface-sampling_amd/csrc/api_painn.hip
--- a/surface-sampling_amd/csrc/api_painn.hip
+++ b/surface-sampling_amd/csrc/api_painn.hip
@@ -189,6 +189,7 @@
         }
         if (const char *e = getenv("VSSR_EDGE_IMPL")) h->edge_impl = (strcmp(e, "gather") == 0) ? 0 : 1;
         if (const char *e = getenv("VSSR_L0_FACTORISE")) h->l0_enabled = h->painn_general ? 0 : atoi(e);
+        if (const char *e = getenv("VSSR_L0_FUSE")) h->l0_fuse = atoi(e);
         if (const char *e = getenv("VSSR_UPD_SAVE")) h->upd_save = atoi(e);
         if (const char *e = getenv("VSSR_DEBUG_KEEP")) h->debug_keep = atoi(e);
         if (const char *e = getenv("VSSR_EDGE_FS16_MAX")) h->fs16_max_atoms = atoi(e);
diff --git a/surface-sampling_amd/csrc/mfma16.h b/surface-sampling_amd/csrc/mfma16.h
--- a/surface-sampling_amd/csrc/mfma16.h
+++ b/surface-sampling_amd/csrc/mfma16.h
@@ -217,5 +217,69 @@
 #endif
 }
 
-}
-#endif
+constexpr int KP = 24;
+constexpr int TBLK = 4 * KP;
+constexpr int L0_TILE_U4 = 1024;
+
+template <bool WEIGHTS_A>
+__device__ __forceinline__ void l0_chunk_mfma(const Planes &Ps, const Planes &Pv, int chunk, int r, int g, const u32x4 (&b)[2][2],
+                                              f32x4 (&acc)[8]) {
+    u32x4 a[8][2];
+#pragma unroll
+    for (int t = 0; t < 8; ++t) {
+        const Planes &P = t < 2 ? Ps : Pv;
+        const int row = (t < 2 ? 16 * t : 16 * (t - 2)) + r;
+        a[t][0] = *reinterpret_cast<const u32x4 *>(P.h + row * P.ld + 32 * chunk + 8 * g);
+        a[t][1] = *reinterpret_cast<const u32x4 *>(P.l + row * P.ld + 32 * chunk + 8 * g);
+    }
+    __builtin_amdgcn_sched_barrier(0);
+#pragma unroll
+    for (int k = 0; k < 3; ++k)
+#pragma unroll
+        for (int t = 0; t < 8; ++t) {
+            const u32x4 wp = b[t < 2 ? 0 : 1][k == 0 ? 1 : 0], ap = a[t][k == 1 ? 1 : 0];
+            acc[t] = WEIGHTS_A ? mfma16(wp, ap, acc[t]) : mfma16(ap, wp, acc[t]);
+            __builtin_amdgcn_sched_barrier(0);
+        }
+}
+
+__device__ __forceinline__ void l0_q_tiles(int m, int a0, int N, int nz, int n_embed, const int *__restrict__ zlist,
+                                           const uint4 *__restrict__ At16, const Planes &Xs, const Planes &Xv,
+                                           float *__restrict__ Q ) {
+    const int lane = threadIdx.x & 63, r = lane & 15, g = lane >> 4, w = threadIdx.x >> 6;
+    for (int ct = w; ct < 2 * nz; ct += NW) {
+        const int q = ct >> 1, hf = ct & 1;
+        const uint4 *wb = At16 + (((size_t)m * n_embed + zlist[q]) * 2) * L0_TILE_U4 + (size_t)hf * 512 + lane;
+        f32x4 acc[8];
+#pragma unroll
+        for (int t = 0; t < 8; ++t) acc[t] = (f32x4){0.f, 0.f, 0.f, 0.f};
+        u32x4 bb[2][2][2];
+        auto load_w = [&](int buf, int c) {
+#pragma unroll
+            for (int sec = 0; sec < 2; ++sec)
+#pragma unroll
+                for (int pc = 0; pc < 2; ++pc) bb[buf][sec][pc] = gload4u(wb + sec * L0_TILE_U4 + (c * 2 + pc) * 64);
+        };
+        load_w(0, 0);
+#pragma unroll
+        for (int c = 0; c < F / 32; ++c) {
+            if (c + 1 < F / 32) load_w((c + 1) & 1, c + 1);
+            l0_chunk_mfma<false>(Xs, Xv, c, r, g, bb[c & 1], acc);
+        }
+        const int kap = 16 * hf + r;
+        if (kap < KP) {
+#pragma unroll
+            for (int t = 0; t < 8; ++t) {
+                const int comp = t < 2 ? 0 : 1 + (t - 2) / 2, tt = t < 2 ? t : (t - 2) & 1;
+#pragma unroll
+                for (int i = 0; i < 4; ++i) {
+                    const int a_ = a0 + 16 * tt + 4 * g + i;
+                    if (a_ < N) Q[((((size_t)m * N + a_) * nz + q) * 4 + comp) * KP + kap] = acc[t][i];
+                }
+            }
+        }
+    }
+}
+
+}
+#endif
diff --git a/surface-sampling_amd/csrc/painn.hip b/surface-sampling_amd/csrc/painn.hip
--- a/surface-sampling_amd/csrc/painn.hip
+++ b/surface-sampling_amd/csrc/painn.hip
@@ -566,6 +566,17 @@
         VSSR_HIP(h, hipMemsetAsync(h->d_sat.p, 0, h->d_sat.bytes, h->stream));
         VSSR_HIP(h, hipMemsetAsync(h->d_sat_out.p, 0, h->d_sat_out.bytes, h->stream));
     }
+    return VSSR_OK;
+}
+
+int painn_materialise_l0_adjoints(vssr_handle *h) {
+    if (!h->l0_adjoints_pending) return VSSR_OK;
+    const StateView &sv = h->sv;
+    const ActiveView av{h->active_mask, h->d_atom_cfg.as<int>(), h->d_sat.as<unsigned>()};
+    launch_update_bwd_mfma(h->stream, h->n_atoms, h->n_models, 0, 2, 0, av, h->model_table.as<ModelW>(), sv.s_msg[0], sv.v_msg[0],
+                           h->l0_sbar_up, sv.vbar, sv.s_in[1], sv.phibar, nullptr, nullptr, sv.sbar_msg_l0, sv.vbar_msg, nullptr);
+    VSSR_HIP(h, hipStreamSynchronize(h->stream));
+    h->l0_adjoints_pending = false;
     return VSSR_OK;
 }
 
@@ -621,6 +632,14 @@
     const bool keep = h->upd_save && (want & VSSR_WANT_FORCES) && readout_mfma_supported(H);
     auto save_of = [&](int l) -> void * { return keep ? (char *)h->d_upd_save.p + update_save_bytes(N, M) * (size_t)l : nullptr; };
     h->l0_used = l0_fact;
+    const bool l0_fused_bwd = l0_fact && h->l0_fuse && h->l0T_by_geom && L >= 2 && !h->debug_keep && !h->upd_save &&
+                              (want & VSSR_WANT_FORCES) && readout_mfma_supported(H);
+    L0Tail l0v;
+    if (l0_fused_bwd) {
+        rc = l0_prepare(h, &l0v);
+        if (rc) return rc;
+    }
+    h->l0_adjoints_pending = false;
 
     if (!l0_fact) {
         P.begin(KC_EMBED, st);
@@ -690,16 +709,24 @@
             else if (l == L - 1)
                 launch_update_bwd_mfma(st, N, M, l, 1, 1, av, MW, sv.s_msg[l], sv.v_msg[l], nullptr, sv.vbar, sv.s_in[L], nullptr,
                                        e_excl, sv.e_atom, sbar_msg_l, sv.vbar_msg, save_of(l));
-            else
+            else if (l == 0 && l0_fused_bwd) {
+                launch_update_bwd_l0_mfma(st, N, M, av, MW, sv.s_msg[0], sv.v_msg[0], sbar_msg_up, sv.vbar, sv.s_in[1], sv.phibar, l0v);
+                h->l0_adjoints_pending = true;
+                h->l0_sbar_up = sbar_msg_up;
+            } else
                 launch_update_bwd_mfma(st, N, M, l, 2, 0, av, MW, sv.s_msg[l], sv.v_msg[l], sbar_msg_up, sv.vbar, sv.s_in[l + 1],
                                        sv.phibar, nullptr, nullptr, sbar_msg_l, sv.vbar_msg, save_of(l));
             P.end(st);
             sv.sbar_msg_l0 = sbar_msg_l;
+            if (l == 0 && l0_fact && !l0_fused_bwd) {
+                P.begin(KC_L0_BWD, st);
+                l0_run_q(h, G, sbar_msg_l, sv.vbar_msg);
+                P.end(st);
+            }
             P.begin((l == 0 && l0_fact) ? KC_L0_BWD : KC_EDGE_BWD, st);
             int accumulate = (l != L - 1);
             if (l == 0 && l0_fact) {
-                rc = l0_run_reverse(h, G, (int)(L == 1), (int)compact, sbar_msg_l, sv.vbar_msg, sv.gbar, (long long)h->slot_cap,
-                                    fin_groups);
+                rc = l0_run_reverse(h, G, (int)(L == 1), (int)compact, sv.gbar, (long long)h->slot_cap, fin_groups);
                 if (rc) return rc;
             } else if (l == 0)
                 hipLaunchKernelGGL(k_edge_bwd<true>, g_atom, blk, 0, st, N, l, accumulate, MW, G, counters,
diff --git a/surface-sampling_amd/csrc/painn_l0.hip b/surface-sampling_amd/csrc/painn_l0.hip
--- a/surface-sampling_amd/csrc/painn_l0.hip
+++ b/surface-sampling_amd/csrc/painn_l0.hip
@@ -2,8 +2,6 @@
 
 namespace vssr {
 
-constexpr int KP = 24;
-constexpr int TBLK = 4 * KP;
 
 template <int NZ>
 __global__ void __launch_bounds__(96)
@@ -55,7 +53,6 @@
     for (int z = 0; z < NZ; ++z) T[((size_t)i * nz + z) * TBLK + comp * KP + kap] = acc[z];
 }
 
-constexpr int L0_TILE_U4 = 1024;
 
 __global__ void __launch_bounds__(NTHREADS)
 k_l0_fwd16(int N, int M, int nz, ActiveView av, const int *__restrict__ counters, const int *__restrict__ Z,
@@ -94,7 +91,7 @@
         for (int t = 0; t < 8; ++t) acc[t] = (f32x4){0.f, 0.f, 0.f, 0.f};
 #pragma unroll 1
         for (int q = 0; q < nz; ++q) {
-            u32x4 b[2][2], a[8][2];
+            u32x4 b[2][2];
 #pragma unroll
             for (int sec = 0; sec < 2; ++sec)
 #pragma unroll
@@ -103,21 +100,7 @@
                 const int qn = q + 1 < nz ? q + 1 : 0, mn = q + 1 < nz ? m : m + 1;
                 if (mn < M) load_w(mn, qn);
             }
-#pragma unroll
-            for (int t = 0; t < 8; ++t) {
-                const Planes &P = t < 2 ? Ts : Tv;
-                const int row = (t < 2 ? 16 * t : 16 * (t - 2)) + r;
-                a[t][0] = *reinterpret_cast<const u32x4 *>(P.h + row * P.ld + 32 * q + 8 * g);
-                a[t][1] = *reinterpret_cast<const u32x4 *>(P.l + row * P.ld + 32 * q + 8 * g);
-            }
-            __builtin_amdgcn_sched_barrier(0);
-#pragma unroll
-            for (int k = 0; k < 3; ++k)
-#pragma unroll
-                for (int t = 0; t < 8; ++t) {
-                    acc[t] = mfma16(b[t < 2 ? 0 : 1][k == 0 ? 1 : 0], a[t][k == 1 ? 1 : 0], acc[t]);
-                    __builtin_amdgcn_sched_barrier(0);
-                }
+            l0_chunk_mfma<true>(Ts, Tv, q, r, g, b, acc);
         }
 #pragma unroll
         for (int t = 0; t < 2; ++t) {
@@ -149,55 +132,7 @@
     }, sat);
     sat.commit(av, a0, N);
     __syncthreads();
-    const int lane = threadIdx.x & 63, r = lane & 15, g = lane >> 4, w = threadIdx.x >> 6;
-    for (int ct = w; ct < 2 * nz; ct += NW) {
-        const int q = ct >> 1, hf = ct & 1;
-        const uint4 *wb = At16 + (((size_t)m * n_embed + zlist[q]) * 2) * L0_TILE_U4 + (size_t)hf * 512 + lane;
-        f32x4 acc[8];
-#pragma unroll
-        for (int t = 0; t < 8; ++t) acc[t] = (f32x4){0.f, 0.f, 0.f, 0.f};
-        u32x4 bb[2][2][2];
-        auto load_w = [&](int buf, int c) {
-#pragma unroll
-            for (int sec = 0; sec < 2; ++sec)
-#pragma unroll
-                for (int pc = 0; pc < 2; ++pc) bb[buf][sec][pc] = gload4u(wb + sec * L0_TILE_U4 + (c * 2 + pc) * 64);
-        };
-        load_w(0, 0);
-#pragma unroll
-        for (int c = 0; c < F / 32; ++c) {
-            u32x4 (&b)[2][2] = bb[c & 1];
-            u32x4 a[8][2];
-            if (c + 1 < F / 32) load_w((c + 1) & 1, c + 1);
-#pragma unroll
-            for (int t = 0; t < 8; ++t) {
-                const Planes &P = t < 2 ? Xs : Xv;
-                const int row = (t < 2 ? 16 * t : 16 * (t - 2)) + r;
-                a[t][0] = *reinterpret_cast<const u32x4 *>(P.h + row * P.ld + 32 * c + 8 * g);
-                a[t][1] = *reinterpret_cast<const u32x4 *>(P.l + row * P.ld + 32 * c + 8 * g);
-            }
-            __builtin_amdgcn_sched_barrier(0);
-#pragma unroll
-            for (int k = 0; k < 3; ++k)
-#pragma unroll
-                for (int t = 0; t < 8; ++t) {
-                    acc[t] = mfma16(a[t][k == 1 ? 1 : 0], b[t < 2 ? 0 : 1][k == 0 ? 1 : 0], acc[t]);
-                    __builtin_amdgcn_sched_barrier(0);
-                }
-        }
-        const int kap = 16 * hf + r;
-        if (kap < KP) {
-#pragma unroll
-            for (int t = 0; t < 8; ++t) {
-                const int comp = t < 2 ? 0 : 1 + (t - 2) / 2, tt = t < 2 ? t : (t - 2) & 1;
-#pragma unroll
-                for (int i = 0; i < 4; ++i) {
-                    const int a_ = a0 + 16 * tt + 4 * g + i;
-                    if (a_ < N) Q[((((size_t)m * N + a_) * nz + q) * 4 + comp) * KP + kap] = acc[t][i];
-                }
-            }
-        }
-    }
+    l0_q_tiles(m, a0, N, nz, n_embed, zlist, At16, Xs, Xv, Q);
 }
 
 __global__ void __launch_bounds__(256)
@@ -331,12 +266,25 @@
     return VSSR_OK;
 }
 
+int l0_prepare(vssr_handle *h, L0Tail *tail) {
+    const int N = h->n_atoms, M = h->n_models, nz = h->l0_nz;
+    if (h->d_l0T.ensure(sizeof(float) * (size_t)N * nz * TBLK) ||
+        h->d_l0Q.ensure(sizeof(float) * (size_t)M * N * nz * TBLK))
+        return set_err(h, VSSR_E_NOMEM, "layer-0 factorisation buffers: out of device memory");
+    if (tail) {
+        tail->nz = nz;
+        tail->n_embed = h->n_embed;
+        tail->zlist = h->d_zlist.as<int>();
+        tail->At16 = h->d_l0At.as<uint4>();
+        tail->Q = h->d_l0Q.as<float>();
+    }
+    return VSSR_OK;
+}
+
 int l0_run_forward(vssr_handle *h, const GraphView &G, float *s_msg, float *v_msg) {
     const int N = h->n_atoms, M = h->n_models, nz = h->l0_nz;
     hipStream_t st = h->stream;
-    if (h->d_l0T.ensure(sizeof(float) * (size_t)N * nz * TBLK) ||
-        h->d_l0Q.ensure(sizeof(float) * (size_t)M * N * nz * TBLK))
-        return set_err(h, VSSR_E_NOMEM, "layer-0 factorisation buffers: out of device memory");
+    if (int rc = l0_prepare(h, nullptr)) return rc;
     if (!h->l0T_by_geom) {
         const int *cnt = h->d_counters.as<int>();
         float *T = h->d_l0T.as<float>();
@@ -358,13 +306,16 @@
     return VSSR_OK;
 }
 
-int l0_run_reverse(vssr_handle *h, const GraphView &G, int first_write, int fresh_mfma, const float *sbar_msg, const float *vbar_msg,
-                   float4 *gbar, long long gbar_stride, int n_groups) {
+void l0_run_q(vssr_handle *h, const GraphView &G, const float *sbar_msg, const float *vbar_msg) {
+    const int N = h->n_atoms, M = h->n_models, nz = h->l0_nz;
+    const size_t lds_q = sizeof(_Float16) * (plane_halves(TA, F) + plane_halves(3 * TA, F));
+    hipLaunchKernelGGL(k_l0_q16, dim3((N + TA - 1) / TA, M), dim3(NTHREADS), lds_q, h->stream, N, nz, G.act, h->d_counters.as<int>(),
+                       h->d_zlist.as<int>(), h->d_l0At.as<uint4>(), h->n_embed, sbar_msg, vbar_msg, h->d_l0Q.as<float>());
+}
+
+int l0_run_reverse(vssr_handle *h, const GraphView &G, int first_write, int fresh_mfma, float4 *gbar, long long gbar_stride, int n_groups) {
     const int N = h->n_atoms, M = h->n_models, nz = h->l0_nz;
     hipStream_t st = h->stream;
-    const size_t lds_q = sizeof(_Float16) * (plane_halves(TA, F) + plane_halves(3 * TA, F));
-    hipLaunchKernelGGL(k_l0_q16, dim3((N + TA - 1) / TA, M), dim3(NTHREADS), lds_q, st, N, nz, G.act, h->d_counters.as<int>(),
-                       h->d_zlist.as<int>(), h->d_l0At.as<uint4>(), h->n_embed, sbar_msg, vbar_msg, h->d_l0Q.as<float>());
     if (sizeof(float) * 4 * M * nz * TBLK > 48 * 1024)
         VSSR_HIP(h, hipFuncSetAttribute((const void *)k_l0_bwd, hipFuncAttributeMaxDynamicSharedMemorySize, 160 * 1024));
     hipLaunchKernelGGL(k_l0_bwd, dim3((N + 3) / 4), dim3(256), sizeof(float) * 4 * M * nz * TBLK, st, N, M, nz, first_write, fresh_mfma,
diff --git a/surface-sampling_amd/csrc/painn_node_mfma.hip b/surface-sampling_amd/csrc/painn_node_mfma.hip
--- a/surface-sampling_amd/csrc/painn_node_mfma.hip
+++ b/surface-sampling_amd/csrc/painn_node_mfma.hip
@@ -695,8 +695,9 @@
                   const float *__restrict__ v_msg, const float *__restrict__ sbar_src, const float *__restrict__ vbar,
                   const float *__restrict__ s_next, const float *__restrict__ phibar, const float *__restrict__ e_excl,
                   float *__restrict__ e_atom, float *__restrict__ sbar_msg, float *__restrict__ vbar_msg,
-                  const f32x4 *__restrict__ save) {
+                  const f32x4 *__restrict__ save, L0Tail l0) {
     static_assert(!SAVED || RT == 2, "the saved layout is that of the 32-atom forward kernel");
+    static_assert(MODE != 3 || (RT == 2 && !SAVED), "the layer-0 tail works on 32-atom tiles and recomputes the block");
     extern __shared__ __attribute__((aligned(16))) _Float16 ldsh[];
     constexpr int TA = 16 * RT, OFF_VT = UpdLds<RT>::OFF_VT, OFF_AS = UpdLds<RT>::OFF_AS, UPD_LDS_HALVES = UpdLds<RT>::HALVES;
     const int m = blockIdx.y, a0 = blockIdx.x * TA;
@@ -925,6 +926,29 @@
     PH(31)
     __syncthreads();
     PH(32)
+    if constexpr (MODE == 3) {
+        const Planes Xs = make_planes(ldsh, TA, F), Xv = make_planes(ldsh + plane_halves(TA, F), 3 * TA, F);
+        static_assert(plane_halves(TA, F) + plane_halves(3 * TA, F) <= UPD_LDS_HALVES, "adjoint planes stay in front of the vbar tile");
+        {
+            SatTrack satq;
+#pragma unroll
+            for (int t = 0; t < RT; ++t) {
+                const int row = L.row(t);
+                store_split4(Xs, row, L.col0, sb[t] + hbar[t][0], satq);
+#pragma unroll
+                for (int x = 0; x < 3; ++x) {
+                    f32x4 r = {0.f, 0.f, 0.f, 0.f};
+                    if (!vbar_is_zero) r = *reinterpret_cast<const f32x4 *>(VB + (x * TA + row) * FT + L.col0);
+                    store_split4(Xv, x * TA + row, L.col0, r + out[RT * x + t][0], satq);
+                }
+            }
+            satq.commit(av, a0, N);
+        }
+        __syncthreads();
+        l0_q_tiles(m, a0, N, l0.nz, l0.n_embed, l0.zlist, l0.At16, Xs, Xv, l0.Q);
+        PH(33)
+        return;
+    }
     float *T = reinterpret_cast<float *>(ldsh);
 #pragma unroll
     for (int t = 0; t < RT; ++t) {
@@ -1002,7 +1026,7 @@
 #define SET_UPD(MODE)                                                                                                     \
     VSSR_HIP(h, hipFuncSetAttribute((const void *)k_update_bwd_mfma<MODE, 2>, hipFuncAttributeMaxDynamicSharedMemorySize, \
                                     (int)node_mfma_lds_bytes(3)));
-    SET_UPD(0) SET_UPD(1) SET_UPD(2)
+    SET_UPD(0) SET_UPD(1) SET_UPD(2) SET_UPD(3)
 #undef SET_UPD
     VSSR_HIP(h, hipFuncSetAttribute((const void *)k_update_bwd_mfma<1, 2, true>, hipFuncAttributeMaxDynamicSharedMemorySize,
                                     (int)node_mfma_lds_bytes(3)));
@@ -1059,10 +1083,10 @@
         (void)once;
         if (mode == 1)
             hipLaunchKernelGGL((k_update_bwd_mfma<1, 1, false>), grid1, blk1, lds1, st, N, l, vbar_is_zero, av, MW, s_msg, v_msg, sbar_src,
-                               vbar, s_next, phibar, e_excl, e_atom, sbar_msg, vbar_msg, sv);
+                               vbar, s_next, phibar, e_excl, e_atom, sbar_msg, vbar_msg, sv, L0Tail());
         else
             hipLaunchKernelGGL((k_update_bwd_mfma<2, 1, false>), grid1, blk1, lds1, st, N, l, vbar_is_zero, av, MW, s_msg, v_msg, sbar_src,
-                               vbar, s_next, phibar, e_excl, e_atom, sbar_msg, vbar_msg, sv);
+                               vbar, s_next, phibar, e_excl, e_atom, sbar_msg, vbar_msg, sv, L0Tail());
         return;
     }
 #endif
@@ -1070,11 +1094,18 @@
     const size_t lds = node_mfma_lds_bytes(3);
 #define LAUNCH_UPD(MODE, SAVED)                                                                                             \
     hipLaunchKernelGGL((k_update_bwd_mfma<MODE, 2, SAVED>), grid, blk, lds, st, N, l, vbar_is_zero, av, MW, s_msg, v_msg, sbar_src, \
-                       vbar, s_next, phibar, e_excl, e_atom, sbar_msg, vbar_msg, sv)
+                       vbar, s_next, phibar, e_excl, e_atom, sbar_msg, vbar_msg, sv, L0Tail())
     if (mode == 1) { if (sv) LAUNCH_UPD(1, true); else LAUNCH_UPD(1, false); }
     else if (mode == 2) { if (sv) LAUNCH_UPD(2, true); else LAUNCH_UPD(2, false); }
     else LAUNCH_UPD(0, false);
 #undef LAUNCH_UPD
 }
-
-}
+void launch_update_bwd_l0_mfma(hipStream_t st, int N, int M, const ActiveView &av, const ModelW *MW, const float *s_msg,
+                               const float *v_msg, const float *sbar_src, const float *vbar, const float *s_next, const float *phibar,
+                               const L0Tail &l0) {
+    hipLaunchKernelGGL((k_update_bwd_mfma<3, 2, false>), dim3((N + TA - 1) / TA, M), dim3(NTHREADS), node_mfma_lds_bytes(3), st, N, 0, 0,
+                       av, MW, s_msg, v_msg, sbar_src, vbar, s_next, phibar, (const float *)nullptr, (float *)nullptr, (float *)nullptr,
+                       (float *)nullptr, (const f32x4 *)nullptr, l0);
+}
+
+}
diff --git a/surface-sampling_amd/csrc/vssr_internal.h b/surface-sampling_amd/csrc/vssr_internal.h
--- a/surface-sampling_amd/csrc/vssr_internal.h
+++ b/surface-sampling_amd/csrc/vssr_internal.h
@@ -52,6 +52,13 @@
             if (mask[c]) return true;
         return false;
     }
+};
+
+struct L0Tail {
+    int nz = 0, n_embed = 0;
+    const int *zlist = nullptr;
+    const uint4 *At16 = nullptr;
+    float *Q = nullptr;
 };
 
 struct GraphView {
@@ -332,6 +339,9 @@
     vssr::DevBuf d_hits;
     int l0_enabled = 1, l0_nz = 0;
     bool l0_used = false;
+    int l0_fuse = 1;
+    const float *l0_sbar_up = nullptr;
+    bool l0_adjoints_pending = false;
     vssr::DevBuf d_l0A, d_l0At;
     vssr::DevBuf d_zmap, d_zlist;
     vssr::DevBuf d_l0T, d_l0Q;
@@ -485,6 +495,9 @@
                             const float *s_msg, const float *v_msg, const float *sbar_src, const float *vbar,
                             const float *s_next, const float *phibar, const float *e_excl, float *e_atom,
                             float *sbar_msg, float *vbar_msg, const void *save);
+void launch_update_bwd_l0_mfma(hipStream_t st, int N, int M, const ActiveView &av, const ModelW *MW, const float *s_msg,
+                               const float *v_msg, const float *sbar_src, const float *vbar, const float *s_next, const float *phibar,
+                               const L0Tail &l0);
 void pack_mfma_tiles16(const float *Wsrc, int rows, int K, unsigned *dst );
 void build_wd16(const float *Wd, const float *bd, unsigned *dst );
 void l0_build_tables(const float *blob_embed, const float *W1, const float *b1, const float *W2, const float *b2,
@@ -492,9 +505,11 @@
 void l0_pack_tables(const float *A, int n_embed, unsigned *A16, unsigned *At16);
 size_t l0_packed_dwords(int n_embed);
 int l0_mfma_init(vssr_handle *h);
+int painn_materialise_l0_adjoints(vssr_handle *h);
+int l0_prepare(vssr_handle *h, L0Tail *tail);
 int l0_run_forward(vssr_handle *h, const GraphView &G, float *s_msg, float *v_msg);
-int l0_run_reverse(vssr_handle *h, const GraphView &G, int first_write, int fresh_mfma, const float *sbar_msg, const float *vbar_msg,
-                   float4 *gbar, long long gbar_stride, int n_groups);
+void l0_run_q(vssr_handle *h, const GraphView &G, const float *sbar_msg, const float *vbar_msg);
+int l0_run_reverse(vssr_handle *h, const GraphView &G, int first_write, int fresh_mfma, float4 *gbar, long long gbar_stride, int n_groups);
 int edge_mfma_init(vssr_handle *h);
 enum { EDGE_CLASS_FS16 = 0, EDGE_CLASS_FS16M = 1, EDGE_CLASS_FS8 = 2, EDGE_CLASS_FS4 = 3, EDGE_CLASS_GATHER = 4, EDGE_CLASSES = 5,
        EDGE_MFMA_CLASSES = 4 };
```

Result: faster. 24940 evaluations/s, median of 6 (+1.2%).
